# zhouxuguang/GNXRayTracer

Hardware: AMD Instinct MI355X
Metric: Mrays/sec + wall-clock to 1024spp, dragon Cornell 1920×1080 (higher is better)
Workload: dtype f32; 1 GPU; cfg3: Cornell + synthetic 100000-tri mesh (stand-in for absent dragon.3d), Glass+Metal, PathIntegrator maxDepth 8 rr 1 spatial, Halton(1024), 1920x1080; passes_in_flight=4, sub_passes=56, spp_rendered=1024, gather=n/a, world_size=1, backend=none, devices_visible=1

## Files before the change

### gnxraytracer_amd/__init__.py

```python
import collections
import ctypes as C
import os

import numpy as np

from . import _abi
from ._abi import (Camera, Hit, Light, LiSample, Material, Medium, Ray, RenderParams, SceneDesc, Stats, Texture)
from ._tensors import (ANY_GPU, SOME, _addr, _arrays_on_device, _edit_stream, _expect, _got, _host_or_device, _image, _image_size, _is_tensor, _is_torch, _only_kw,
                       _out_tensor, _outputs, _ptr, _refuse, _same_count, _stream_handle, _stream_pair)

_HERE = os.path.dirname(os.path.abspath(__file__))
LIB_PATH = os.environ.get("GNXR_LIB", os.path.join(_HERE, "libgnxr.so"))


class GnxrError(RuntimeError):
    pass


_lib = None
_device = 0


def lib():
    global _lib
# ... 212 lines not shown
        return _check(lib().gnxr_builder_add_sphere(self._h, c, float(radius), int(material), int(medium_inside), int(medium_outside)))

    def set_camera(self, eye=(0, 0, 5), look=(0, 0, 0), up=(0, 1, 0), fov=90.0, lens_radius=0.0, focal_distance=3.0, orthographic=False):
        cam = Camera(_f3(eye), _f3(look), _f3(up), fov, lens_radius, focal_distance, int(bool(orthographic)))
        _check(lib().gnxr_builder_set_camera(self._h, C.byref(cam)))

    def set_bvh_split_method(self, method):
        _check(lib().gnxr_builder_set_bvh_split_method(self._h, {"sah": 0, "hlbvh": 1, "middle": 2, "equal_counts": 3}[method]))

    def set_camera_medium(self, medium):
        _check(lib().gnxr_builder_set_camera_medium(self._h, int(medium)))

    def desc(self):
        d = SceneDesc()
        _check(lib().gnxr_builder_desc(self._h, C.byref(d)))
        return d


def camera(eye=(0, 0, 5), look=(0, 0, 0), up=(0, 1, 0), fov=90.0, lens_radius=0.0, focal_distance=3.0, orthographic=False):
    return Camera(_f3(eye), _f3(look), _f3(up), fov, lens_radius, focal_distance, int(bool(orthographic)))


def _material_albedo(m):
    rgb = (C.c_float * 3)()
    _check(lib().gnxr_material_albedo(C.byref(m), rgb))
    return np.array(rgb[:], dtype=np.float32)


def material_albedo(**material_fields):
    return _material_albedo(material(**material_fields))


def material(**material_fields):
    m = Material()
    for k, v in material_fields.items():
        if isinstance(v, (tuple, list, np.ndarray)):
            setattr(m, k, (C.c_float * len(v))(*[float(x) for x in v]))
        else:
            setattr(m, k, v)
    return m


def write_synthetic_3d(path, target_triangles=100000, seed=1):
    _check(lib().gnxr_write_synthetic_3d(os.fsencode(path), int(target_triangles), int(seed)))


class Scene:

    def __init__(self, builder_or_desc):
        self._h = C.c_void_p()
        self._keep = builder_or_desc
        d = builder_or_desc.desc() if isinstance(builder_or_desc, SceneBuilder) else builder_or_desc
        self.n_triangles = int(d.n_triangles)
        self.n_vertices = int(d.n_vertices)
        self.n_lights = int(d.n_lights)
        self.device = _device
        self.camera = Camera()
        C.memmove(C.byref(self.camera), C.byref(d.camera), C.sizeof(Camera))
        self._env_light = None
        for i in range(int(d.n_lights)):
            if d.lights[i].type == _abi.LIGHT_INFINITE:
                self._env_light = Light()
                C.memmove(C.byref(self._env_light), C.byref(d.lights[i]), C.sizeof(Light))
                break
        self._textures = []
        for i in range(int(d.n_textures)):
            t = Texture()
            C.memmove(C.byref(t), C.byref(d.textures[i]), C.sizeof(Texture))
            t.texel_offset = 0
            self._textures.append(t)
        _check(lib().gnxr_scene_create(C.byref(d), C.byref(self._h)))

    def close(self):
        if getattr(self, "_h", None) and _lib is not None:
            _lib.gnxr_scene_destroy(self._h)
            self._h = None

    __del__ = close

    def info(self):
        n, dmax, nv = C.c_int32(), C.c_int32(), C.c_int32()
        _check(lib().gnxr_scene_info(self._h, C.byref(n), C.byref(dmax), C.byref(nv)))
        return {"bvh_nodes": n.value, "bvh_max_depth": dmax.value, "light_voxels": nv.value}

    def nee_apply_counts(self):
        t, w = C.c_uint64(), C.c_uint64()
        _check(lib().gnxr_scene_nee_apply_counts(self._h, C.byref(t), C.byref(w)))
        return int(t.value), int(w.value)

    def update_vertices(self, xyz, first_vertex=0, stream=None, move_lights=False):
        ptr, xyz, _ = _host_or_device("update_vertices", xyz, np.float32, [(None, 3)], "(n, 3)", self.device)
        stream = _stream_handle("update_vertices", _edit_stream(stream, xyz))
        if move_lights:
            _check(lib().gnxr_scene_update_vertices_ex(self._h, int(first_vertex), int(xyz.shape[0]), _addr(ptr), _abi.UPDATE_MOVE_LIGHTS, _addr(stream)))
        else:
            _check(lib().gnxr_scene_update_vertices(self._h, int(first_vertex), int(xyz.shape[0]), _addr(ptr), _addr(stream)))

    def update_lights(self, lights, first_light=0):
        lights = list(lights)
        for l in lights:
            if not isinstance(l, Light):
                raise ValueError(f"update_lights: lights must be gnxr Light records, got {type(l).__name__}")
        arr = (Light * max(len(lights), 1))(*lights)
        _check(lib().gnxr_scene_update_lights(self._h, int(first_light), len(lights), arr))

    def set_lights(self, lights, stream=None):
        lights = list(lights)
        for l in lights:
            if not isinstance(l, Light):
                raise ValueError(f"set_lights: lights must be gnxr Light records, got {type(l).__name__}")
        handle = _stream_handle("set_lights", stream)
        arr = (Light * max(len(lights), 1))()
        for k, l in enumerate(lights):
            C.memmove(C.byref(arr[k]), C.byref(l), C.sizeof(Light))
        _check(lib().gnxr_scene_set_lights(self._h, arr if lights else None, len(lights), _addr(handle)))
        self.n_lights = len(lights)
        self._env_light = None
        for l in lights:
            if l.type == _abi.LIGHT_INFINITE:
                self._env_light = Light()
                C.memmove(C.byref(self._env_light), C.byref(l), C.sizeof(Light))
                break

    def light_tables(self):
        out = []
        for which, dtype, cols in ((0, np.uint32, _abi.DLIGHT_BYTES // 4), (1, np.int32, 0)):
            n = C.c_int64(0)
            _check(lib().gnxr_scene_light_tables(self._h, which, None, 0, C.byref(n)))
            a = np.zeros(n.value // 4, dtype)
            if n.value:
                _check(lib().gnxr_scene_light_tables(self._h, which, C.c_void_p(a.ctypes.data), n.value, C.byref(n)))
            out.append(a.reshape(-1, cols) if cols else a)
        return tuple(out)

    def update_materials(self, materials, first_material=0):
        materials = list(materials)
        for m in materials:
            if not isinstance(m, Material):
                raise ValueError(f"update_materials: materials must be gnxr Material records, got {type(m).__name__}")
        arr = (Material * max(len(materials), 1))(*materials)
        _check(lib().gnxr_scene_update_materials(self._h, int(first_material), len(materials), arr))

    def set_triangle_materials(self, ids, first_triangle=0, stream=None):
        ptr, ids, _ = _host_or_device("set_triangle_materials", ids, np.int32, [(None,)], "(n,)", self.device)
        stream = _stream_handle("set_triangle_materials", _edit_stream(stream, ids))
        _check(lib().gnxr_scene_set_triangle_materials(self._h, int(first_triangle), int(ids.shape[0]), _addr(ptr), _addr(stream)))

    def triangle_materials(self):
        mat = np.zeros(self.n_triangles, np.int32); cls = np.zeros(self.n_triangles, np.uint8)
        rc = lib().gnxr_scene_triangle_materials(self._h, mat.ctypes.data_as(C.POINTER(C.c_int32)), cls.ctypes.data_as(C.POINTER(C.c_uint8)), self.n_triangles)
        if rc < 0:
            _check(rc)
        return mat, cls

    def update_attributes(self, uv=None, normals=None, tangents=None, first_triangle=0, stream=None):
        name = "update_attributes"
        given = [(what, x, cols) for what, x, cols in (("uv", uv, 6), ("normals", normals, 9), ("tangents", tangents, 9)) if x is not None]
        if not given:
            raise ValueError(f"{name}: none of uv, normals, tangents given")
        on_device = _arrays_on_device(name, given[0][0], given[0][1])
        handle = _stream_handle(name, _edit_stream(stream, given[0][1]))
        ptrs, keep, n = {}, [], None
        for what, x, cols in given:
            ptrs[what], x, _ = _host_or_device(f"{name}: {what}", x, np.float32, [(None, cols)], f"(n, {cols})", self.device, on_device)
            keep.append(x)
            if n is not None and x.shape[0] != n:
# ... 621 lines not shown
NearLists = collections.namedtuple("NearLists", "count records prim dist2 p b1 b2 feature")
NearLists.__doc__ = """Scene.within's and Scene.nearest's result: `count`, int32 (n,) -- within: all triangles inside the radius, never clamped;
nearest: the slots filled --, `records`, the (n, K, 8) float32 gnxr_closest_point records -- per query the first min(count, K) near
triangles in ascending (dist2, prim), then empty slots (prim -1, dist2 +inf, the rest 0) --, and views of it: `prim` (n, K) (int32:
authoring-order triangle), `dist2` (n, K), `p` (n, K, 3), `b1`, `b2` (n, K) and `feature` (n, K) (int32, as in ClosestPoints)."""

SphereCasts = collections.namedtuple("SphereCasts", "records prim t p b1 b2 feature")
SphereCasts.__doc__ = """Scene.sphere_cast's result: `records`, the (n, 8) float32 gnxr_closest_point records with t in the dist2 slot, and views of
it -- `prim` (int32: the authoring-order triangle the ball touches first, -1 without a hit), `t` (the time of impact in units of the
direction, +inf without a hit), `p` (n, 3), `b1`, `b2` and `feature` (int32, as in ClosestPoints): the contact point on that triangle."""

ALL_HITS_MAX = 32
NEAR_MAX = 32
CONTAINS_DIRECTION = (0.8017837, 0.5345225, 0.26726124)


def rays_tensor(o, d, tmax=float("inf")):
    import torch
    o = torch.as_tensor(o, dtype=torch.float32).reshape(-1, 3)
    d = torch.as_tensor(d, dtype=torch.float32, device=o.device).reshape(-1, 3)
    r = torch.zeros((o.shape[0], 8), dtype=torch.float32, device=o.device)
    r[:, 0:3] = o
    r[:, 3] = torch.as_tensor(tmax, dtype=torch.float32, device=o.device)
    r[:, 4:7] = d
    return r


def _view_args(name, cameras, media, width, height):
    if cameras is not None:
        cameras = list(cameras)
        for c in cameras:
            if not isinstance(c, Camera):
                raise ValueError(f"{name}: cameras must be gnxr Camera records (camera(...)), got {type(c).__name__}")
        if media is not None:
            media = [int(m) for m in media]
            if len(media) != len(cameras):
                raise ValueError(f"{name}: {len(media)} media for {len(cameras)} cameras")
    return (cameras, media) + _image_size(name, width, height)


def li_samples(px, py, s, medium=-1):
    import torch
    args = {"px": px, "py": py, "s": s, "medium": medium}
    device = next((a.device for a in args.values() if isinstance(a, torch.Tensor)), torch.device("cpu"))
    cols = []
    for name, a in args.items():
        if isinstance(a, torch.Tensor):
            if a.dtype.is_floating_point or a.dtype.is_complex or a.dtype == torch.bool or a.dim() > 1:
                raise ValueError(f"li_samples: {name} must be an integer tensor of shape (n,) or (), got {a.dtype} {tuple(a.shape)}")
            a = a.to(device=device, dtype=torch.int32)
        elif isinstance(a, (int, np.integer)) and not isinstance(a, bool):
            a = torch.tensor(int(a), dtype=torch.int32, device=device)
        else:
            raise ValueError(f"li_samples: {name} must be an integer or an integer tensor, got {type(a).__name__}")
        cols.append(a.reshape(-1))
    try:
        cols = torch.broadcast_tensors(*cols)
    except RuntimeError as e:
        raise ValueError(f"li_samples: the arguments do not broadcast: {e}") from None
    return torch.stack(cols, dim=1).contiguous()


HIT_DTYPE = np.dtype([("prim", np.int32), ("t", np.float32), ("b0", np.float32), ("b1", np.float32), ("b2", np.float32),
                      ("n", np.float32, 3)])


CLOSEST_DTYPE = np.dtype([("prim", np.int32), ("dist2", np.float32), ("p", np.float32, 3), ("b1", np.float32), ("b2", np.float32),
                          ("feature", np.int32)])


RAY_HIT_DTYPE = np.dtype([("t", np.float32), ("prim", np.int32), ("b1", np.float32), ("b2", np.float32)])


def make_rays(o, d, tmax=np.inf):
    o = np.asarray(o, dtype=np.float32).reshape(-1, 3)
    d = np.asarray(d, dtype=np.float32).reshape(-1, 3)
    r = np.zeros((len(o), 8), dtype=np.float32)
    r[:, 0:3] = o
    r[:, 3] = tmax
    r[:, 4:7] = d
    return r


def stats_dict(s):
    return {k: getattr(s, k) for k, _ in Stats._fields_}


class PathIntegrator:
    integrator = _abi.INTEGRATOR_PATH

    def __init__(self, maxDepth=5, rrThreshold=1.0, lightSampleStrategy="spatial"):
        self.maxDepth = int(maxDepth)
        self.rrThreshold = float(rrThreshold)
        self.strategy = LIGHT_STRATEGIES.get(lightSampleStrategy, _abi.LIGHTS_SPATIAL)

    def params(self, width, height, spp, spp_begin=0, spp_end=0, shard_index=0, shard_count=1, shard_rows=1,
               samples_per_pass=0, passes_in_flight=0):
        return RenderParams(width, height, spp, spp_begin, spp_end, self.maxDepth, self.rrThreshold, self.integrator,
                            self.strategy, shard_index, shard_count, shard_rows, samples_per_pass, getattr(self, "directStrategy", 0),
                            passes_in_flight)

    def Li(self, scene, rays, samples, width, height, spp, out=None, stream=None, **kw):
        import torch
        _expect("Li: rays", rays, torch.float32, (8,))
        _expect("Li: samples", samples, torch.int32, (4,))
        n = rays.shape[0]
        _same_count("Li", None, samples.shape[0], n, "rays", "sample records")
        out = _out_tensor("Li: out", out, (n, 4), torch.float32, rays.device)
        _expect("Li: rays", rays, torch.float32, (8,), scene.device)
        _expect("Li: samples", samples, torch.int32, (4,), scene.device)
        stream, _ = _stream_pair(stream, rays.device)
        p = self.params(width, height, spp, **kw)
        st = Stats()
        _check(lib().gnxr_li_device(scene._h, C.byref(p), _ptr(rays), _ptr(samples), n, _ptr(out), _addr(stream), C.byref(st)))
        return out, stats_dict(st)

    def RenderViews(self, scene, cameras, width, height, spp, media=None, out=None, stream=None, **kw):
        import torch
        cameras, media, width, height = _view_args("RenderViews", list(cameras), media, width, height)
        V = len(cameras)
        out = _out_tensor("RenderViews: out", out, (V, height, width, 4), torch.float32, torch.device("cuda", scene.device))
        stream, _ = _stream_pair(stream, out.device)
        p = self.params(width, height, spp, **kw)
        cams = (Camera * max(V, 1))(*cameras)
        med = (C.c_int32 * max(V, 1))(*media) if media is not None else None
        st = Stats()
        _check(lib().gnxr_render_views_device(scene._h, C.byref(p), cams, med, V, _ptr(out), _addr(stream), C.byref(st)))
        return out, stats_dict(st)

    def RenderAdaptive(self, scene, width, height, spp, threshold, min_spp=16, step_spp=16, floor=0.01, guard=1, out=None, count_out=None, stream=None, **kw):
        import math
        import torch
        width, height, spp, min_spp, step_spp, guard = int(width), int(height), int(spp), int(min_spp), int(step_spp), int(guard)
        threshold, floor = float(threshold), float(floor)
        _image_size("RenderAdaptive", width, height)
        if spp < 1 or not 1 <= min_spp <= spp:
            raise ValueError(f"RenderAdaptive: spp >= 1 and min_spp in [1, spp] are required, got spp = {spp}, min_spp = {min_spp}")
        if step_spp < 1:
            raise ValueError(f"RenderAdaptive: step_spp must be at least 1, got {step_spp}")
        if not 0 <= guard <= 8:
            raise ValueError(f"RenderAdaptive: guard must lie in [0, 8], got {guard}")
        if math.isnan(threshold) or threshold < 0 or math.isnan(floor) or floor < 0:
            raise ValueError(f"RenderAdaptive: threshold and floor must be numbers >= 0, got {threshold} and {floor}")
        _only_kw("RenderAdaptive", kw, ("samples_per_pass", "passes_in_flight"))
        hstream, _, out, count_out = _outputs(stream, torch.device("cuda", scene.device), ("RenderAdaptive: out", out, (height, width, 4), torch.float32),
                                              ("RenderAdaptive: count_out", count_out, (height, width), torch.int32))
        p = self.params(width, height, spp, **kw)
        ap = _abi.AdaptiveParams(C.sizeof(_abi.AdaptiveParams), min_spp, step_spp, guard, threshold, floor)
        info = _abi.AdaptiveInfo(C.sizeof(_abi.AdaptiveInfo), 0, 0, 0)
        st = Stats()
        _check(lib().gnxr_render_adaptive_device(scene._h, C.byref(p), C.byref(ap), _ptr(out), _ptr(count_out), _addr(hstream), C.byref(st), C.byref(info)))
        stats = stats_dict(st)
        stats.update(rounds=info.rounds, samples=info.samples, pixels_at_budget=info.pixels_at_budget)
        return out, count_out, stats

    AOV_CHANNELS = ("albedo", "normal", "shading_normal", "depth", "ids")

    def RenderAOV(self, scene, width, height, spp, cameras=None, media=None, channels=AOV_CHANNELS, out=None, stream=None, **kw):
        import torch
        channels = tuple(channels)
        bad = [c for c in channels if c not in self.AOV_CHANNELS]
        if bad or not channels or len(set(channels)) != len(channels):
            raise ValueError(f"RenderAOV: channels must be a non-empty selection of {self.AOV_CHANNELS}, got {channels}")
        if cameras is None and media is not None:
            raise ValueError("RenderAOV: media goes with cameras; the scene's own camera sits in the scene's camera medium")
        cameras, media, width, height = _view_args("RenderAOV", cameras, media, width, height)
        V = len(cameras) if cameras is not None else 1
        _only_kw("RenderAOV", kw, ("spp_begin", "spp_end", "samples_per_pass"))
        device = torch.device("cuda", scene.device)
        lead = (V,) if cameras is not None else ()
        shapes = {"albedo": (4,), "normal": (4,), "shading_normal": (4,), "depth": (), "ids": (2,)}
        out = dict(out) if out is not None else {}
        extra = [c for c in out if c not in channels]
        if extra:
            raise ValueError(f"RenderAOV: out holds {extra}, which channels does not name")
        hstream, _, *tensors = _outputs(stream, device, *((f"RenderAOV: out[{c!r}]", out.get(c), lead + (height, width) + shapes[c], torch.int32 if c == "ids" else torch.float32)
                                                           for c in channels))
        res = dict(zip(channels, tensors))
        bufs = _abi.AovBuffers(*(_ptr(res.get(c)) for c in self.AOV_CHANNELS))
        p = self.params(width, height, spp, **kw)
        cams = (Camera * V)(*cameras) if cameras else None
        med = (C.c_int32 * V)(*media) if media else None
        st = Stats()
        _check(lib().gnxr_render_aov_device(scene._h, C.byref(p), cams, med, V if cameras is not None else 1, C.byref(bufs), _addr(hstream), C.byref(st)))
        return res, stats_dict(st)

    def RenderDenoised(self, scene, width, height, spp, cameras=None, media=None, normal="shading_normal", stream=None, **denoise_kw):
        import torch
        spp = int(spp)
        if spp < 2 or spp % 2:
            raise ValueError(f"RenderDenoised: spp must be even and at least 2 (the two halves are the variance estimate), got {spp}")
        if normal not in ("shading_normal", "normal"):
            raise ValueError(f"RenderDenoised: normal must be 'shading_normal' or 'normal', got {normal!r}")
        if cameras is None and media is not None:
            raise ValueError("RenderDenoised: media goes with cameras; the scene's own camera sits in the scene's camera medium")
        _only_kw("RenderDenoised", denoise_kw, ("iterations", "sigma_color", "sigma_normal", "sigma_depth", "out"))
        cameras, media, width, height = _view_args("RenderDenoised", cameras, media, width, height)
        device = torch.device("cuda", scene.device)
        hstream, tstream = _stream_pair(stream, device)
        halves, stats = [], []
        for lo, hi in ((0, spp // 2), (spp // 2, spp)):
            if cameras is not None:
                img, st = self.RenderViews(scene, cameras, width, height, spp, media=media, stream=tstream, spp_begin=lo, spp_end=hi)
            else:
                with torch.cuda.stream(tstream):
                    img = torch.zeros((height, width, 4), dtype=torch.float32, device=device)
                st = self.RenderDevice(scene, img.data_ptr(), width, height, spp, stream=hstream, spp_begin=lo, spp_end=hi)
            halves.append(img)
            stats.append(st)
        aov, aov_stats = self.RenderAOV(scene, width, height, spp, cameras=cameras, media=media, channels=("albedo", normal, "depth"), stream=tstream)
        image = denoise(halves[0], halves[1], albedo=aov["albedo"], normal=aov[normal], depth=aov["depth"], stream=tstream, **denoise_kw)
        total = {k: stats[0][k] + stats[1][k] for k in stats[0]}
        total["aov"] = aov_stats
        return image, total

    def RenderFiltered(self, scene, width, height, spp, filter, cameras=None, media=None, accum=None, resume=False, out=None, stream=None, **kw):
        import torch
        _film_record("RenderFiltered", filter, "filter must be")
        if cameras is None and media is not None:
            raise ValueError("RenderFiltered: media goes with cameras; the scene's own camera sits in the scene's camera medium")
        cameras, media, width, height = _view_args("RenderFiltered", cameras, media, width, height)
        if resume and accum is None:
            raise ValueError("RenderFiltered: resume continues an accumulator: pass the tensor of the earlier call as accum")
        _only_kw("RenderFiltered", kw, ("spp_begin", "spp_end", "samples_per_pass", "passes_in_flight"))
        V = len(cameras) if cameras is not None else 1
        shape = ((V,) if cameras is not None else ()) + (height, width, 4)
        given = [("RenderFiltered: accum", accum, shape, torch.float32)] if accum is not None else []
        hstream, *_, out = _outputs(stream, torch.device("cuda", scene.device), *given, ("RenderFiltered: out", out, shape, torch.float32))
        p = self.params(width, height, spp, **kw)
        cams = (Camera * V)(*cameras) if cameras else None
        med = (C.c_int32 * V)(*media) if media else None
        st = Stats()
        _check(lib().gnxr_render_filtered_device(scene._h, C.byref(p), C.byref(filter), cams, med, V, _ptr(out), _ptr(accum), _abi.FILM_CONTINUE if resume else 0,
                                                 _addr(hstream), C.byref(st)))
        return out, stats_dict(st)

    def BakeLightmap(self, scene, lm_uv, width, height, spp, dilate=2, flip=False, medium=-1, out=None, stream=None, **kw):
        import torch
        width, height = _image_size("BakeLightmap", width, height, "atlas")
        if int(dilate) < 0:
            raise ValueError(f"BakeLightmap: dilate must be >= 0, got {dilate}")
        _only_kw("BakeLightmap", kw, ("samples_per_pass", "passes_in_flight"))
        _bake_uv("BakeLightmap", scene, lm_uv)
        hstream, _, out = _outputs(stream, lm_uv.device, ("BakeLightmap: out", out, (height, width, 4), torch.float32))
        p = self.params(width, height, spp, **kw)
        bp = _abi.BakeParams(C.sizeof(_abi.BakeParams), _abi.BAKE_FLIP_NORMALS if flip else 0, int(dilate), int(medium))
        st = Stats()
        _check(lib().gnxr_bake_lightmap_device(scene._h, C.byref(p), C.byref(bp), _ptr(lm_uv), _ptr(out), _addr(hstream), C.byref(st)))
        return out, stats_dict(st)

    def BakeLightProbes(self, scene, positions, spp, width=None, height=None, medium=-1, out=None, stream=None, **kw):
        import torch
        _expect("BakeLightProbes: positions", positions, torch.float32, (3,), scene.device)
        n = positions.shape[0]
        if width is None:
            width = max(1, min(n, 1024))
        width = int(width)
        if height is None:
            height = max(1, -(-n // width)) if width > 0 else 0
        height = int(height)
        if width <= 0 or height <= 0 or width * height < n:
            raise ValueError(f"BakeLightProbes: the {width} x {height} grid of pixels does not hold {n} probes")
        _only_kw("BakeLightProbes", kw, ("samples_per_pass", "passes_in_flight"))
        hstream, _, out = _outputs(stream, positions.device, ("BakeLightProbes: out", out, (n, 9, 4), torch.float32))
        p = self.params(width, height, spp, **kw)
        pp = _abi.LightprobeParams(C.sizeof(_abi.LightprobeParams), 0, int(medium))
        st = Stats()
        _check(lib().gnxr_bake_lightprobes_device(scene._h, C.byref(p), C.byref(pp), _ptr(positions), n, _ptr(out), _addr(hstream), C.byref(st)))
        return out, stats_dict(st)

    def Render(self, scene, width, height, spp, **kw):
        p = self.params(width, height, spp, **kw)
        img = np.zeros((height, width, 4), dtype=np.float32)
        st = Stats()
        _check(lib().gnxr_render(scene._h, C.byref(p), img.ctypes.data_as(C.POINTER(C.c_float)), C.byref(st)))
        return img, stats_dict(st)

    def Reserve(self, scene, width, height, spp, **kw):
        p = self.params(width, height, spp, **kw)
        _check(lib().gnxr_render_reserve(scene._h, C.byref(p)))

    def RenderDevice(self, scene, d_ptr, width, height, spp, stream=None, **kw):
        p = self.params(width, height, spp, **kw)
        st = Stats()
        _check(lib().gnxr_render_device(scene._h, C.byref(p), C.c_void_p(int(d_ptr)),
                                        C.c_void_p(int(stream) if stream else None), C.byref(st)))
        return stats_dict(st)


class VolPathIntegrator(PathIntegrator):
    integrator = _abi.INTEGRATOR_VOLPATH


class WhittedIntegrator(PathIntegrator):
    integrator = _abi.INTEGRATOR_WHITTED

    def __init__(self, maxDepth=5):
        super().__init__(maxDepth, 1.0, "uniform")


class DirectLightingIntegrator(PathIntegrator):
    integrator = _abi.INTEGRATOR_DIRECT

    def __init__(self, strategy="all", maxDepth=5):
        super().__init__(maxDepth, 1.0, "uniform")
        self.directStrategy = {"all": _abi.DIRECT_SAMPLE_ALL, "one": _abi.DIRECT_SAMPLE_ONE}[strategy]


def sample_halton(width, height, px, py, s, dim):
    px = np.ascontiguousarray(px, dtype=np.int32)
    py = np.ascontiguousarray(py, dtype=np.int32)
    s = np.ascontiguousarray(s, dtype=np.int64)
    dim = np.ascontiguousarray(dim, dtype=np.int32)
    out = np.zeros(len(px), dtype=np.float32)
    _check(lib().gnxr_sample_halton(width, height, px.ctypes.data_as(C.POINTER(C.c_int32)),
                                    py.ctypes.data_as(C.POINTER(C.c_int32)), s.ctypes.data_as(C.POINTER(C.c_int64)),
                                    dim.ctypes.data_as(C.POINTER(C.c_int32)), len(px),
                                    out.ctypes.data_as(C.POINTER(C.c_float))))
    return out


def camera_rays(camera, width, height, px, py, s):
    px = np.ascontiguousarray(px, dtype=np.int32)
    py = np.ascontiguousarray(py, dtype=np.int32)
    s = np.ascontiguousarray(s, dtype=np.int64)
    o = np.zeros((len(px), 3), dtype=np.float32)
    d = np.zeros((len(px), 3), dtype=np.float32)
    _check(lib().gnxr_camera_rays(C.byref(camera), width, height, px.ctypes.data_as(C.POINTER(C.c_int32)),
                                  py.ctypes.data_as(C.POINTER(C.c_int32)), s.ctypes.data_as(C.POINTER(C.c_int64)),
                                  len(px), o.ctypes.data_as(C.POINTER(C.c_float)),
                                  d.ctypes.data_as(C.POINTER(C.c_float))))
    return o, d


def camera_rays_device(camera, width, height, px, py, s, medium=-1, stream=None):
    import torch
    for what, x in (("px", px), ("py", py), ("s", s)):
        if not _is_tensor(x, torch.int32, (None,), ANY_GPU if x is px else px.device):
            _refuse(x, f"camera_rays_device: {what} must be a contiguous int32 (n,) tensor on one GPU")
        _same_count("camera_rays_device", what, x.shape[0], px.shape[0], "px", "entries")
    n = px.shape[0]
    if not isinstance(camera, Camera):
        raise ValueError(f"camera_rays_device: camera must be a gnxr Camera record (camera(...)), got {type(camera).__name__}")
    st, _, rays, samples = _outputs(stream, px.device, ("camera_rays_device: rays", None, (n, 8), torch.float32), ("camera_rays_device: samples", None, (n, 4), torch.int32))
    _check(lib().gnxr_camera_rays_device(C.byref(camera), int(medium), int(width), int(height), _ptr(px), _ptr(py), _ptr(s), n, _ptr(rays), _ptr(samples), _addr(st)))
    return rays, samples


def denoise(color, color_b=None, albedo=None, normal=None, depth=None, iterations=5, sigma_color=4.0, sigma_normal=0.25, sigma_depth=0.01, out=None, stream=None):
    import math
    import torch
    shape, V, H, W = _image("denoise", "color", color, size=False)
    for what, x, want in (("color_b", color_b, shape), ("albedo", albedo, shape), ("normal", normal, shape), ("depth", depth, shape[:-1])):
        if x is not None and not _is_tensor(x, torch.float32, want, color.device):
            _refuse(x, f"denoise: {what} must be a contiguous float32 tensor of shape {want} on {color.device}")
    _image_size("denoise", W, H)
    iterations = int(iterations)
    if not 1 <= iterations <= 8:
        raise ValueError(f"denoise: iterations must lie in [1, 8], got {iterations}")
    sigmas = [float(sigma_color), float(sigma_normal), float(sigma_depth)]
    if any(math.isnan(s) or s < 0 for s in sigmas):
        raise ValueError(f"denoise: the sigmas must be numbers >= 0, got {sigmas}")
    hstream, _, out = _outputs(stream, color.device, ("denoise: out", out, shape, torch.float32))
    if V == 0:
        return out
    p = _abi.DenoiseParams(C.sizeof(_abi.DenoiseParams), W, H, V, iterations, *sigmas)
    bufs = _abi.DenoiseBuffers(C.sizeof(_abi.DenoiseBuffers), 0, _ptr(color), _ptr(color_b), _ptr(albedo), _ptr(normal), _ptr(depth))
    _check(lib().gnxr_denoise_device(C.byref(p), C.byref(bufs), _ptr(out), _addr(hstream)))
    return out

# ... 482 lines not shown
```

### gnxraytracer_amd/_abi.py

```python
import ctypes as C

GNXR_ABI_VERSION = 5

OK, ERR_INVALID, ERR_NO_DEVICE, ERR_OOM, ERR_UNSUPPORTED, ERR_IO, ERR_RUNTIME = 0, -1, -2, -3, -4, -5, -6
MAT_NONE, MAT_MATTE, MAT_MIRROR, MAT_GLASS, MAT_METAL, MAT_PLASTIC, MAT_DISNEY = range(7)
LIGHT_AREA_TRI, LIGHT_INFINITE, LIGHT_SKYBOX, LIGHT_POINT, LIGHT_SPOT, LIGHT_DISTANT = 1, 2, 3, 4, 5, 6
INTEGRATOR_PATH, INTEGRATOR_VOLPATH, INTEGRATOR_WHITTED, INTEGRATOR_DIRECT = 0, 1, 2, 3
DIRECT_SAMPLE_ALL, DIRECT_SAMPLE_ONE = 0, 1
LIGHTS_SPATIAL, LIGHTS_UNIFORM, LIGHTS_POWER = 0, 1, 2
MEDIUM_HOMOGENEOUS, MEDIUM_GRID = 1, 2
NEAR_ALL, NEAR_NEAREST = 0, 1
DMEDIUM_BYTES = 128
DLIGHT_BYTES = 112
DTEXTURE_BYTES = 112
UPDATE_MOVE_LIGHTS = 1

f32, i32, u8, i64, u32, u64 = C.c_float, C.c_int32, C.c_uint8, C.c_int64, C.c_uint32, C.c_uint64


class Material(C.Structure):
    _fields_ = [
        ("type", i32), ("has_bump", i32), ("remap_roughness", i32), ("disney_thin", i32),
        ("kd", f32 * 3), ("ks", f32 * 3), ("kr", f32 * 3), ("kt", f32 * 3), ("eta", f32 * 3), ("k", f32 * 3),
        ("sigma", f32), ("urough", f32), ("vrough", f32),
# ... 153 lines not shown


class MotionParams(C.Structure):
    _fields_ = [("struct_size", i32), ("width", i32), ("height", i32), ("n_views", i32)]


class MotionBuffers(C.Structure):
    _fields_ = [("struct_size", i32), ("_pad", i32), ("d_motion", C.c_void_p), ("d_guide", C.c_void_p), ("d_prim", C.c_void_p)]


class TemporalParams(C.Structure):
    _fields_ = [("struct_size", i32), ("width", i32), ("height", i32), ("n_views", i32), ("max_history", i32), ("depth_tol", f32), ("normal_cos", f32)]


class TemporalBuffers(C.Structure):
    _fields_ = [("struct_size", i32), ("_pad", i32), ("d_color", C.c_void_p), ("d_motion", C.c_void_p), ("d_guide", C.c_void_p), ("d_prim", C.c_void_p),
                ("d_hist_color", C.c_void_p), ("d_hist_stat", C.c_void_p), ("d_hist_guide", C.c_void_p), ("d_hist_prim", C.c_void_p),
                ("d_out_color", C.c_void_p), ("d_out_stat", C.c_void_p)]


class HistogramParams(C.Structure):
    _fields_ = [("struct_size", i32), ("width", i32), ("height", i32), ("n_views", i32), ("min_log2", i32)]


class ExposureParams(C.Structure):
    _fields_ = [("struct_size", i32), ("n_views", i32), ("min_log2", i32), ("_pad", i32), ("key", f32), ("low", f32), ("high", f32), ("rate", f32),
                ("min_exposure", f32), ("max_exposure", f32)]


class TonemapParams(C.Structure):
    _fields_ = [("struct_size", i32), ("width", i32), ("height", i32), ("n_views", i32), ("curve", i32), ("flags", u32), ("exposure", f32), ("white", f32)]


HISTOGRAM_WORDS = 260
TONEMAP_LINEAR, TONEMAP_REFERENCE, TONEMAP_REINHARD, TONEMAP_ACES = range(4)
TONEMAP_SRGB, TONEMAP_ROUND = 1, 2

class SkinParams(C.Structure):
    _fields_ = [("struct_size", i32), ("n_vertices", i32), ("n_bones", i32), ("n_morphs", i32)]


NORMALS_FLIP = 1

FILTER_BOX, FILTER_TRIANGLE, FILTER_GAUSSIAN, FILTER_MITCHELL, FILTER_TABLE = range(5)
FILM_CONTINUE = 1

P = C.POINTER
VP = C.c_void_p

PROTOTYPES = {
    "gnxr_abi_version": (C.c_int, []),
    "gnxr_abi_sizeof": (C.c_int, [C.c_int]),
    "gnxr_init": (C.c_int, [C.c_int]),
    "gnxr_shutdown": (None, []),
    "gnxr_last_error": (C.c_char_p, []),
    "gnxr_init_devices": (C.c_int, [i32, P(i32)]),
    "gnxr_set_profiling": (C.c_int, [C.c_int]),
    "gnxr_probe_valu_peak": (C.c_int, [P(C.c_double)]),
    "gnxr_probe_gather_peak": (C.c_int, [P(C.c_double)]),
    "gnxr_scene_create": (C.c_int, [P(SceneDesc), P(VP)]),
    "gnxr_scene_destroy": (None, [VP]),
    "gnxr_scene_info": (C.c_int, [VP, P(i32), P(i32), P(i32)]),
    "gnxr_scene_update_vertices": (C.c_int, [VP, i32, i32, VP, VP]),
    "gnxr_scene_update_vertices_ex": (C.c_int, [VP, i32, i32, VP, u32, VP]),
    "gnxr_scene_update_lights": (C.c_int, [VP, i32, i32, P(Light)]),
    "gnxr_scene_set_lights": (C.c_int, [VP, P(Light), i32, VP]),
    "gnxr_scene_light_tables": (C.c_int, [VP, i32, VP, i64, P(i64)]),
    "gnxr_scene_rebuild_bvh": (C.c_int, [VP, VP]),
    "gnxr_scene_set_geometry": (C.c_int, [VP, P(Geometry), VP]),
    "gnxr_scene_update_environment": (C.c_int, [VP, P(Light), VP, i32, i32, VP]),
    "gnxr_scene_env_tables": (C.c_int, [VP, i32, VP, i64, P(i64)]),
    "gnxr_scene_update_media": (C.c_int, [VP, i32, i32, P(Medium), VP, VP]),
    "gnxr_scene_media_tables": (C.c_int, [VP, i32, i32, VP, i64, P(i64)]),
    "gnxr_scene_update_textures": (C.c_int, [VP, i32, i32, P(Texture), VP, VP]),
    "gnxr_scene_texture_tables": (C.c_int, [VP, i32, i32, VP, i64, P(i64)]),
    "gnxr_scene_update_materials": (C.c_int, [VP, i32, i32, P(Material)]),
    "gnxr_scene_set_triangle_materials": (C.c_int, [VP, i32, i32, VP, VP]),
    "gnxr_scene_triangle_materials": (C.c_int, [VP, P(i32), P(C.c_uint8), C.c_int64]),
    "gnxr_scene_set_camera": (C.c_int, [VP, P(Camera), i32]),
    "gnxr_render": (C.c_int, [VP, P(RenderParams), P(f32), P(Stats)]),
    "gnxr_render_device": (C.c_int, [VP, P(RenderParams), VP, VP, P(Stats)]),
    "gnxr_render_reserve": (C.c_int, [VP, P(RenderParams)]),
    "gnxr_scene_nee_apply_counts": (C.c_int, [VP, P(u64), P(u64)]),
    "gnxr_trace_closest": (C.c_int, [VP, P(Ray), i64, P(Hit)]),
    "gnxr_trace_any": (C.c_int, [VP, P(Ray), i64, P(u8)]),
    "gnxr_trace_closest_device": (C.c_int, [VP, VP, i64, VP, VP]),
    "gnxr_trace_any_device": (C.c_int, [VP, VP, i64, VP, VP]),
    "gnxr_closest_point_device": (C.c_int, [VP, VP, i64, VP, VP]),
    "gnxr_closest_point_counted_device": (C.c_int, [VP, VP, i64, VP, VP, VP]),
    "gnxr_closest_point": (C.c_int, [VP, P(PointQuery), i64, P(ClosestPoint)]),
    "gnxr_trace_all_device": (C.c_int, [VP, VP, i64, i32, VP, VP, VP]),
    "gnxr_trace_all_counted_device": (C.c_int, [VP, VP, i64, i32, VP, VP, VP, VP]),
    "gnxr_trace_all": (C.c_int, [VP, P(Ray), i64, i32, P(RayHit), P(i32)]),
    "gnxr_near_device": (C.c_int, [VP, VP, i64, i32, u32, VP, VP, VP]),
    "gnxr_near_counted_device": (C.c_int, [VP, VP, i64, i32, u32, VP, VP, VP, VP]),
    "gnxr_near": (C.c_int, [VP, P(PointQuery), i64, i32, u32, P(ClosestPoint), P(i32)]),
    "gnxr_sphere_cast_device": (C.c_int, [VP, VP, i64, VP, VP]),
    "gnxr_sphere_cast_counted_device": (C.c_int, [VP, VP, i64, VP, VP, VP]),
    "gnxr_sphere_cast": (C.c_int, [VP, P(SphereCast), i64, P(ClosestPoint)]),
    "gnxr_li_device": (C.c_int, [VP, P(RenderParams), VP, VP, i64, VP, VP, P(Stats)]),
    "gnxr_render_views_device": (C.c_int, [VP, P(RenderParams), P(Camera), P(i32), i32, VP, VP, P(Stats)]),
    "gnxr_render_aov_device": (C.c_int, [VP, P(RenderParams), P(Camera), P(i32), i32, P(AovBuffers), VP, P(Stats)]),
    "gnxr_render_adaptive_device": (C.c_int, [VP, P(RenderParams), P(AdaptiveParams), VP, VP, VP, P(Stats), P(AdaptiveInfo)]),
    "gnxr_denoise_device": (C.c_int, [P(DenoiseParams), P(DenoiseBuffers), VP, VP]),
    "gnxr_film_filter_table": (C.c_int, [P(FilmFilter), P(f32)]),
    "gnxr_film_add_device": (C.c_int, [P(FilmFilter), i32, i32, i32, i32, VP, VP, VP, VP]),
    "gnxr_film_resolve_device": (C.c_int, [i32, i32, i32, VP, VP, VP]),
    "gnxr_render_filtered_device": (C.c_int, [VP, P(RenderParams), P(FilmFilter), P(Camera), P(i32), i32, VP, VP, u32, VP, P(Stats)]),
    "gnxr_bake_texels_device": (C.c_int, [VP, VP, i32, i32, VP, VP, VP]),
    "gnxr_surface_rays_device": (C.c_int, [VP, i32, i32, VP, VP, VP, VP, VP, i64, u32, i32, VP, VP, VP, VP]),
    "gnxr_bake_dilate_device": (C.c_int, [i32, i32, i32, VP, VP]),
    "gnxr_bake_lightmap_device": (C.c_int, [VP, P(RenderParams), P(BakeParams), VP, VP, VP, P(Stats)]),
    "gnxr_lightprobe_rays_device": (C.c_int, [VP, i32, i32, VP, VP, VP, VP, i64, i32, VP, VP, VP]),
    "gnxr_sh_project_device": (C.c_int, [VP, VP, i32, i64, VP, u32, VP]),
    "gnxr_bake_lightprobes_device": (C.c_int, [VP, P(RenderParams), P(LightprobeParams), VP, i32, VP, VP, P(Stats)]),
    "gnxr_sh_irradiance_device": (C.c_int, [VP, i32, VP, VP, i64, VP, VP]),
    "gnxr_camera_matrices": (C.c_int, [P(Camera), i32, i32, P(f32), P(f32), P(f32)]),
    "gnxr_motion_device": (C.c_int, [VP, P(MotionParams), P(Camera), P(Camera), VP, P(MotionBuffers), VP]),
    "gnxr_temporal_accumulate_device": (C.c_int, [P(TemporalParams), P(TemporalBuffers), VP]),
    "gnxr_luminance_histogram_device": (C.c_int, [P(HistogramParams), VP, VP, VP]),
    "gnxr_exposure_device": (C.c_int, [P(ExposureParams), VP, VP, VP, VP]),
    "gnxr_tonemap_device": (C.c_int, [P(TonemapParams), VP, VP, VP, VP]),
    "gnxr_scene_update_attributes": (C.c_int, [VP, i32, i32, VP, VP, VP, VP]),
    "gnxr_scene_triangle_attributes": (C.c_int, [VP, i32, P(f32), i64, P(i64)]),
    "gnxr_scene_recompute_normals": (C.c_int, [VP, u32, VP]),
    "gnxr_skin_vertices_device": (C.c_int, [P(SkinParams), VP, VP, VP, VP, VP, VP, VP, VP]),
    "gnxr_material_albedo": (C.c_int, [P(Material), P(f32)]),
    "gnxr_camera_rays_device": (C.c_int, [P(Camera), i32, i32, i32, VP, VP, VP, i64, VP, VP, VP]),
    "gnxr_bsdf_device": (C.c_int, [VP, VP, VP, VP, VP, i64, i32, VP, VP]),
    "gnxr_light_sample_device": (C.c_int, [VP, VP, i64, i32, VP, VP]),
    "gnxr_light_le_device": (C.c_int, [VP, i32, VP, i64, VP, VP]),
    "gnxr_sample_halton": (C.c_int, [i32, i32, P(i32), P(i32), P(i64), P(i32), i64, P(f32)]),
    "gnxr_camera_rays": (C.c_int, [P(Camera), i32, i32, P(i32), P(i32), P(i64), i64, P(f32), P(f32)]),
    "gnxr_framebuffer_update": (C.c_int, [P(f32), P(f32), i32, i32, i32, P(u8)]),
    "gnxr_framebuffer_save_png": (C.c_int, [C.c_char_p, P(u8), i32, i32]),
    "gnxr_light_grid_table": (C.c_int, [VP, i32, i32, P(f32), i64, P(i64)]),
    "gnxr_eval_libm": (C.c_int, [i32, P(f32), P(f32), i64, P(f32)]),
    "gnxr_eval_libm_f64": (C.c_int, [i32, P(f32), i64, P(C.c_double)]),
    "gnxr_builder_create": (C.c_int, [P(VP)]),
    "gnxr_builder_set_camera_medium": (C.c_int, [VP, i32]),
    "gnxr_builder_add_sphere": (C.c_int, [VP, P(f32), f32, i32, i32, i32]),
    "gnxr_builder_destroy": (None, [VP]),
    "gnxr_builder_add_material": (C.c_int, [VP, P(Material)]),
    "gnxr_builder_matte": (C.c_int, [VP, P(f32), f32]),
    "gnxr_builder_mirror": (C.c_int, [VP, P(f32)]),
    "gnxr_builder_purple_plastic": (C.c_int, [VP]),
    "gnxr_builder_yellow_metal": (C.c_int, [VP]),
    "gnxr_builder_white_glass": (C.c_int, [VP]),
    "gnxr_builder_add_mesh": (C.c_int, [VP, P(f32), i32, P(i32), i32, P(f32), i32, i32, i32]),
    "gnxr_builder_add_model_3d": (C.c_int, [VP, C.c_char_p, i32]),
    "gnxr_builder_add_cornell": (C.c_int, [VP, i32, i32, i32]),
    "gnxr_builder_add_floor": (C.c_int, [VP, i32]),
    "gnxr_builder_add_area_light": (C.c_int, [VP, i32]),
    "gnxr_builder_add_sky_light": (C.c_int, [VP]),
    "gnxr_builder_add_inf_light": (C.c_int, [VP, C.c_char_p]),
    "gnxr_builder_add_inf_light_data": (C.c_int, [VP, P(f32), i32, i32, P(f32), P(f32)]),
    "gnxr_builder_add_medium": (C.c_int, [VP, P(Medium), P(f32)]),
    "gnxr_builder_add_volume_file": (C.c_int, [VP, C.c_char_p, f32, f32, P(f32)]),
    "gnxr_builder_add_emissive_mesh": (C.c_int, [VP, P(f32), i32, P(i32), i32, P(f32), i32, P(f32), i32]),
    "gnxr_builder_add_spot_light": (C.c_int, [VP]),
    "gnxr_builder_add_dist_light": (C.c_int, [VP]),
    "gnxr_builder_add_light": (C.c_int, [VP, P(Light)]),
    "gnxr_builder_add_texture_data": (C.c_int, [VP, P(Texture), P(f32), i32, i32]),
    "gnxr_builder_add_texture_file": (C.c_int, [VP, P(Texture), C.c_char_p]),
    "gnxr_builder_set_material_texture": (C.c_int, [VP, i32, i32, i32]),
    "gnxr_builder_set_triangle_uv": (C.c_int, [VP, i32, i32, P(f32)]),
# ... 22 lines not shown
```

### gnxraytracer_amd/csrc/api.hip

```cpp
#include <hip/hip_runtime.h>

#include <chrono>
#include <cstdio>
#include <cstdlib>
#include <memory>
#include <mutex>
#include <string>
#include <thread>
#include <vector>

#include "host_scene.h"
#include "kernels.hip.h"
#include "trace4_kernel.hip.h"
#include "hlbvh_build.hip.h"
#include "refit_kernel.hip.h"
#include "material_kernel.hip.h"
#include "rebuild_kernel.hip.h"
#include "geometry_kernel.hip.h"
#include "lights_kernel.hip.h"
#include "env_build_kernel.hip.h"
#include "media_kernel.hip.h"
#include "texture_build_kernel.hip.h"
#include "li_kernel.hip.h"
#include "views_kernel.hip.h"
// ... 101 lines not shown
    return GNXR_OK;
}
#endif
#ifdef GX_TAIL_STAMP
int gnxr_debug_tail_stamp(unsigned long long *out12, int reset) {
    if (hipMemcpyFromSymbol(out12, HIP_SYMBOL(g_tail), 12 * sizeof(unsigned long long)) != hipSuccess) return GNXR_ERR_INVALID;
    if (reset) { unsigned long long z[12] = {~0ull, 0ull, ~0ull, 0ull}; (void)hipMemcpyToSymbol(HIP_SYMBOL(g_tail), z, sizeof(z)); }
    return GNXR_OK;
}
#endif

static int upload_scene(gnxr_scene *s, const SceneUploadTables &up) {
    const SceneFacts &cs = s->cs;
    int rc;
    if (cs.bvh_max_depth + 1 > 64) { set_error("BVH depth %d exceeds the 64-entry traversal stack (BVHAccel.cpp:661)", cs.bvh_max_depth); return GNXR_ERR_UNSUPPORTED; }
    s->set_traversal(std::any_of(up.nodes.begin(), up.nodes.end(), [](const DNode &n) { return (n.meta & 0xffffu) > 127; }));
#define UP(from, field) if ((rc = s->field.upload(from.field)) != GNXR_OK) return rc;
    UP(up, nodes) UP(up, nodes4) UP(up, tris) UP(up, leaf_boxes) UP(up, tri_class) UP(cs, lights) UP(cs, perms) UP(cs, primes) UP(cs, prime_sums) UP(cs, prime_magic)
    UP(cs, dmedia) UP(up, grid_density) UP(up, tri_media) UP(cs, spheres) UP(cs, textures) UP(up, tex_texels) UP(up, ewa_lut) UP(up, tri_uv) UP(up, tri_n) UP(up, tri_s)
    UP(cs, aov_albedo)
    UP(cs, env_texels4) UP(cs, env_cond_func) UP(cs, env_cond_cdf) UP(cs, env_cond_int) UP(cs, env_marg_func) UP(cs, env_marg_cdf) UP(cs, env_marg_guide) UP(cs, env_cond_guide)
#undef UP
    {
        const size_t worst = 2 * cs.desc_materials.size();
        if ((rc = s->material_authored.alloc(worst)) || (rc = s->materials.alloc(1 + worst)) || (rc = s->materials_single.alloc(1 + worst))) return rc;
        if ((rc = s->material_authored.upload(cs.material_authored)) != GNXR_OK) return rc;
        const DTexTables at = s->tex_tables(s->tri_uv.p, s->tri_n.p, s->tri_s.p);
        if ((rc = s->write_material_tables(cs.materials, cs.materials_single, at.tri_uv, at.tri_n, at.tri_s)) != GNXR_OK) return rc;
    }
    if ((rc = s->infinite.upload(cs.infinite_lights)) != GNXR_OK) return rc;
    if ((rc = s->counters.alloc(1)) != GNXR_OK) return rc;
    if (hipHostMalloc((void **)&s->h_counters, sizeof(Counters)) != hipSuccess) { set_error("hipHostMalloc failed"); return GNXR_ERR_OOM; }
    if (hipHostMalloc((void **)&s->h_ring, sizeof(Counters) * gnxr_scene::kRing) != hipSuccess) { set_error("hipHostMalloc failed"); return GNXR_ERR_OOM; }
    for (hipEvent_t &e : s->ring_ev) HIP_TRY(hipEventCreateWithFlags(&e, hipEventDisableTiming));
    for (hipStream_t &a : s->aux_stream) HIP_TRY(hipStreamCreateWithFlags(&a, hipStreamNonBlocking));
    HIP_TRY(hipEventCreateWithFlags(&s->ev_fork, hipEventDisableTiming));
    for (hipEvent_t &e : s->ev_join) HIP_TRY(hipEventCreateWithFlags(&e, hipEventDisableTiming));
    return GNXR_OK;
}

int gnxr_scene_create(const gnxr_scene_desc *desc, gnxr_scene **out) {
    if (!desc || !out) { set_error("null argument"); return GNXR_ERR_INVALID; }
    int rc = ensure_device();
    if (rc) return rc;
    gnxr_scene *s = new (std::nothrow) gnxr_scene(g_device);
    if (!s) return GNXR_ERR_OOM;
    CompiledScene compiled;
    if (!compile_scene(desc, &compiled, device_hlbvh_build)) { delete s; return GNXR_ERR_INVALID; }
    s->cs = std::move(static_cast<SceneFacts &>(compiled));
    s->cs.refit_seeds = std::move(static_cast<RefitSeeds &>(compiled));
    for (size_t i = 1; i < g_devices.size(); ++i) s->replicas.push_back(std::make_unique<gnxr_scene>(g_devices[i], s->host));
    s->host->copies_awaiting_seeds = s->n_copies();
    if ((rc = s->each_copy([&](gnxr_scene *c, size_t) { return upload_scene(c, compiled); })) != GNXR_OK) { delete s; return rc; }
    const SceneFacts &cs = s->cs;
    if (getenv("GNXR_VERBOSE"))
        fprintf(stderr, "[gnxr] scene: %zu tris, %zu nodes (depth %d), %zu 4-wide nodes (stack %d), wide=%d, %zu device(s)\n", cs.n_triangles, cs.n_nodes, cs.bvh_max_depth,
                cs.n_nodes4, cs.stack4_need, (int)s->wide_ok, s->n_copies());
    *out = s;
    return GNXR_OK;
}
void gnxr_scene_destroy(gnxr_scene *s) { delete s; }

int gnxr_scene_info(const gnxr_scene *s, int32_t *n_nodes, int32_t *max_depth, int32_t *n_vox) {
    if (!s) return GNXR_ERR_INVALID;
    if (n_nodes) *n_nodes = (int32_t)s->cs.n_nodes;
    if (max_depth) *max_depth = s->cs.bvh_max_depth;
    if (n_vox) *n_vox = s->grid_strategy >= 0 ? s->grid.nvox[0] * s->grid.nvox[1] * s->grid.nvox[2] : 0;
    return GNXR_OK;
}

int gnxr_scene_nee_apply_counts(gnxr_scene *s, uint64_t *in_trace, uint64_t *by_sweep) {
    if (!s) { set_error("null argument"); return GNXR_ERR_INVALID; }
    std::lock_guard<std::recursive_mutex> lock(s->render_mutex);
    uint64_t t = 0, w = 0;
    for (size_t i = 0; i <= s->replicas.size(); ++i) {
        const Counters *c = s->copy(i)->h_counters;
        if (c) { t += c->nee_applied_trace; w += c->nee_applied_sweep; }
    }
    if (in_trace) *in_trace = t;
    if (by_sweep) *by_sweep = w;
    return GNXR_OK;
}

int gnxr_render_device(gnxr_scene *s, const gnxr_render_params *pin, void *d_rgba_out, void *hip_stream, gnxr_stats *stats) {
    return render_sharded(s, pin, d_rgba_out, hip_stream, stats);
}

int gnxr_render_reserve(gnxr_scene *s, const gnxr_render_params *pin) {
    if (!s || !pin) { set_error("null argument"); return GNXR_ERR_INVALID; }
    int dummy = 0;
    return render_sharded(s, pin, &dummy, nullptr, nullptr, true);
}

int gnxr_render(gnxr_scene *s, const gnxr_render_params *p, float *rgba_out, gnxr_stats *stats) {
    if (!s || !p || !rgba_out) { set_error("null argument"); return GNXR_ERR_INVALID; }
    if (p->width <= 0 || p->height <= 0) { set_error("invalid image size"); return GNXR_ERR_INVALID; }
    size_t npx = (size_t)p->width * p->height;
    std::lock_guard<std::recursive_mutex> lock(s->render_mutex);
    if (int brc = s->bind()) return brc;
    const bool grew = !(s->out.p && npx <= s->out.n);
    int rc = s->out.alloc(npx);
    if (rc) return rc;
    HIP_TRY(hipMemset(s->out.p, 0, npx * sizeof(float4)));
    rc = render_sharded(s, p, s->out.p, nullptr, stats);
    if (rc) { if (grew) s->out.release(); return rc; }
    int sc = p->shard_count > 0 ? p->shard_count : 1, sr = p->shard_rows > 0 ? p->shard_rows : 1;
    if (sc == 1) {
        HIP_TRY(hipMemcpy(rgba_out, s->out.p, npx * sizeof(float4), hipMemcpyDeviceToHost));
    } else {
        for (int y = 0; y < p->height; ++y)
            if ((y / sr) % sc == p->shard_index)
                HIP_TRY(hipMemcpy(rgba_out + (size_t)y * p->width * 4, s->out.p + (size_t)y * p->width, (size_t)p->width * sizeof(float4), hipMemcpyDeviceToHost));
    }
    return GNXR_OK;
}

int gnxr_scene_bvh(const gnxr_scene *sc, float *bounds6, int32_t *meta3, int32_t *ordered, int64_t node_capacity, int64_t *n_nodes) {
    if (!sc || !n_nodes) { set_error("bad argument"); return GNXR_ERR_INVALID; }
    gnxr_scene *s = const_cast<gnxr_scene *>(sc);
    std::lock_guard<std::recursive_mutex> lock(s->render_mutex);
    *n_nodes = (int64_t)s->cs.n_nodes;
    if (!bounds6 || !meta3 || !ordered || node_capacity < *n_nodes) return GNXR_OK;
    if (int rc = s->bind()) return rc;
    std::vector<DNode> nodes(s->cs.n_nodes);
    std::vector<DTri> tris(s->cs.n_triangles);
    HIP_TRY(hipMemcpy(nodes.data(), s->nodes.p, nodes.size() * sizeof(DNode), hipMemcpyDeviceToHost));
    HIP_TRY(hipMemcpy(tris.data(), s->tris.p, tris.size() * sizeof(DTri), hipMemcpyDeviceToHost));
    for (size_t i = 0; i < nodes.size(); ++i) {
        const DNode &n = nodes[i];
        bounds6[6 * i + 0] = n.lo[0]; bounds6[6 * i + 1] = n.lo[1]; bounds6[6 * i + 2] = n.lo[2];
        bounds6[6 * i + 3] = n.hi0; bounds6[6 * i + 4] = n.hi1; bounds6[6 * i + 5] = n.hi2;
        const int nPrims = (int)(n.meta & 0xffffu);
        meta3[3 * i + 0] = n.offset; meta3[3 * i + 1] = nPrims; meta3[3 * i + 2] = nPrims ? 0 : (int)(n.meta >> 16);
    }
    for (size_t i = 0; i < tris.size(); ++i) ordered[i] = tris[i].prim;
    return GNXR_OK;
}

int gnxr_trace_closest(gnxr_scene *s, const gnxr_ray *rays, int64_t n, gnxr_hit *hits) {
    if (!s || !rays || !hits || n < 0) { set_error("bad argument"); return GNXR_ERR_INVALID; }
    if (n == 0) return GNXR_OK;
    if (int brc = s->bind()) return brc;
    DevBuf<gnxr_ray> dr;
    DevBuf<gnxr_hit> dh;
    int rc;
    if ((rc = dr.upload(rays, (size_t)n)) || (rc = dh.alloc((size_t)n))) return rc;
    DScene sc = s->device_scene(1, 1);
    if ((rc = binary_trace_api(s, sc, dr.p, n, dh.p, false, nullptr)) != GNXR_OK) return rc;
    HIP_TRY(hipMemcpy(hits, dh.p, (size_t)n * sizeof(gnxr_hit), hipMemcpyDeviceToHost));
    return GNXR_OK;
}
int gnxr_trace_any(gnxr_scene *s, const gnxr_ray *rays, int64_t n, uint8_t *occluded) {
    if (!s || !rays || !occluded || n < 0) { set_error("bad argument"); return GNXR_ERR_INVALID; }
    if (n == 0) return GNXR_OK;
    if (int brc = s->bind()) return brc;
    DevBuf<gnxr_ray> dr;
    DevBuf<unsigned char> dob;
    int rc;
    if ((rc = dr.upload(rays, (size_t)n)) || (rc = dob.alloc((size_t)n))) return rc;
    DScene sc = s->device_scene(1, 1);
    if ((rc = binary_trace_api(s, sc, dr.p, n, dob.p, true, nullptr)) != GNXR_OK) return rc;
    HIP_TRY(hipMemcpy(occluded, dob.p, (size_t)n, hipMemcpyDeviceToHost));
    return GNXR_OK;
}

}
// ... 186 lines not shown
```

### gnxraytracer_amd/csrc/api_common.hip.h

```cpp
#pragma once

namespace { int hip_status(hipError_t e); }
#define HIP_TRY(expr)                                                                                   \
    do {                                                                                                \
        hipError_t e_ = (expr);                                                                         \
        if (e_ != hipSuccess) {                                                                         \
            set_error("%s failed: %s (%s:%d)", #expr, hipGetErrorString(e_), __FILE__, __LINE__);       \
            return hip_status(e_);                                                                      \
        }                                                                                               \
    } while (0)

namespace {

int hip_status(hipError_t e) {
    if (e == hipErrorOutOfMemory) return GNXR_ERR_OOM;
    if (e == hipErrorNoDevice || e == hipErrorInvalidDevice || e == hipErrorInsufficientDriver || e == hipErrorNotInitialized) return GNXR_ERR_NO_DEVICE;
    return GNXR_ERR_RUNTIME;
}

int g_device = -1;
std::vector<int> g_devices;
std::vector<char> g_peer_ok;
int g_num_cus = 256;
int g_profiling = 0;
int g_grid_bpc = 8;
int g_trace_blocks_per_cu = 5;

struct KernelTimer {
    std::vector<hipEvent_t> pool;
    struct Span { int kind; hipEvent_t a, b; };
    std::vector<Span> open;
    size_t used = 0;
    double seconds[3] = {0, 0, 0};
    unsigned launches[3] = {0, 0, 0};
    hipEvent_t get() {
        if (used == pool.size()) { hipEvent_t e; if (hipEventCreate(&e) != hipSuccess) return nullptr; pool.push_back(e); }
        return pool[used++];
    }
    void begin(int kind, hipStream_t st) { Span s{kind, get(), get()}; if (s.a && s.b) { (void)hipEventRecord(s.a, st); open.push_back(s); } }
    void end(hipStream_t st) { if (!open.empty()) (void)hipEventRecord(open.back().b, st); }
    void collect() {
        for (auto &s : open) { float ms = 0; if (hipEventElapsedTime(&ms, s.a, s.b) == hipSuccess) { seconds[s.kind] += ms * 1e-3; launches[s.kind]++; } }
        open.clear();
        used = 0;
    }
    ~KernelTimer() { for (auto e : pool) (void)hipEventDestroy(e); }
};

struct Knobs {
    static int env_int(const char *name, int unset) { const char *e = getenv(name); return e ? atoi(e) : unset; }
    static bool env_set(const char *name) { return getenv(name) != nullptr; }
#define GX_ONCE(type, expr) do { static const type v = (expr); return v; } while (0)
    static int trace_blocks_per_cu() { const int v = env_int("GNXR_TRACE_BLOCKS_PER_CU", 0); return v >= 1 && v <= 8 ? v : 0; }
    static int grid_blocks_per_cu() { const int v = env_int("GNXR_GRID_BLOCKS_PER_CU", 0); return v >= 1 && v <= 4096 ? v : 0; }
    static int trace_lds_levels() { GX_ONCE(int, env_set("GNXR_TRACE_LDS_LEVELS") ? std::max(2, env_int("GNXR_TRACE_LDS_LEVELS", 0)) : 64); }
    static int trace_chunk() { GX_ONCE(int, env_set("GNXR_TRACE_CHUNK") ? std::max(64, env_int("GNXR_TRACE_CHUNK", 0) / 64 * 64) : kTraceChunk); }
    static bool leaf_box_table() { GX_ONCE(bool, env_set("GNXR_LEAF_BOX_TABLE")); }
    static int regions() { GX_ONCE(int, env_int("GNXR_REGIONS", 0)); }
    static bool pipeline() { GX_ONCE(bool, env_int("GNXR_PIPELINE", 1) != 0); }
    static int pipe_cut() { GX_ONCE(int, env_int("GNXR_PIPE_CUT", -1)); }
    static int loop_lag() { GX_ONCE(int, env_int("GNXR_LOOP_LAG", -1)); }
    static int shade_blocks_per_cu() { GX_ONCE(int, env_set("GNXR_SHADE_BLOCKS_PER_CU") ? std::max(1, env_int("GNXR_SHADE_BLOCKS_PER_CU", 0)) : 32); }
    static int shade_lds_dims() { GX_ONCE(int, env_set("GNXR_SHADE_LDS_DIMS") ? std::max(0, std::min(128, env_int("GNXR_SHADE_LDS_DIMS", 0))) : 64); }
    static bool shade_lds_tables() { GX_ONCE(bool, env_int("GNXR_SHADE_LDS_TABLES", 1) != 0); }
    static int shade_streams() { GX_ONCE(int, env_int("GNXR_SHADE_STREAMS", -1)); }
    static bool vol_pack() { GX_ONCE(bool, env_int("GNXR_VOL_PACK", 1) != 0); }
#undef GX_ONCE
    static int volmedia_step_cap() { return env_set("GNXR_VOLMEDIA_STEP_CAP") ? std::max(0, env_int("GNXR_VOLMEDIA_STEP_CAP", 0)) : 64; }
    static bool no_escape_queue() { return env_set("GNXR_NO_ESCAPE_QUEUE"); }
    static bool no_material_queues() { return env_set("GNXR_NO_MATERIAL_QUEUES"); }
    static bool no_narrow_shade() { return env_set("GNXR_NO_NARROW_SHADE"); }
    static bool no_mis_defer() { return env_set("GNXR_NO_MIS_DEFER"); }
    static int mis_defer_step() { const int v = env_int("GNXR_MIS_DEFER_STEP", 2); return v == 1 ? 1 : 2; }
    static int mis_defer_drain_at() { return std::max(1, std::min(64, env_int("GNXR_MIS_DEFER_DRAIN_AT", 64))); }
    static bool no_trace_nee_apply() { return env_set("GNXR_NO_TRACE_NEE_APPLY"); }
    static bool host_light_grid() { return env_set("GNXR_HOST_LIGHT_GRID"); }
    static bool binary_bvh() { return env_set("GNXR_BINARY_BVH"); }
    static long long closest_bin_min() { const char *e = getenv("GNXR_CLOSEST_BIN_MIN"); return e ? std::max(1ll, atoll(e)) : 65536ll; }
    static int closest_lds_levels() { return std::max(1, std::min(24, env_int("GNXR_CLOSEST_LDS_LEVELS", 16))); }
    static int allhits_lds_levels() { return std::max(1, std::min(32, env_int("GNXR_ALLHITS_LDS_LEVELS", 16))); }
    static int near_lds_levels() { return std::max(1, std::min(24, env_int("GNXR_NEAR_LDS_LEVELS", 16))); }
    static int spherecast_lds_levels() { return std::max(1, std::min(24, env_int("GNXR_SPHERECAST_LDS_LEVELS", 16))); }
};

int ensure_device() {
    if (g_device >= 0) { HIP_TRY(hipSetDevice(g_device)); return GNXR_OK; }
    int n = 0;
    hipError_t e = hipGetDeviceCount(&n);
    if (e != hipSuccess || n <= 0) {
        set_error("no HIP device available (%s); libgnxr has no CPU fallback", e != hipSuccess ? hipGetErrorString(e) : "0 devices");
        return GNXR_ERR_NO_DEVICE;
    }
    int dev = 0;
    HIP_TRY(hipGetDevice(&dev));
    hipDeviceProp_t prop;
    HIP_TRY(hipGetDeviceProperties(&prop, dev));
    g_num_cus = prop.multiProcessorCount > 0 ? prop.multiProcessorCount : 256;
    g_device = dev;
    if (const int v = Knobs::trace_blocks_per_cu()) g_trace_blocks_per_cu = v;
    if (const int v = Knobs::grid_blocks_per_cu()) g_grid_bpc = v;
    return GNXR_OK;
}

template <typename T>
struct DevBuf {
    T *p = nullptr;
    size_t n = 0;
    ~DevBuf() { release(); }
    void release() { if (p) { (void)hipFree(p); p = nullptr; n = 0; } }
    int alloc(size_t count) {
        if (count <= n && p) return GNXR_OK;
        release();
        if (count == 0) count = 1;
        HIP_TRY(hipMalloc((void **)&p, count * sizeof(T)));
        n = count;
        return GNXR_OK;
    }
    int upload(const T *src, size_t count) {
        int rc = alloc(count);
        if (rc) return rc;
        if (count) HIP_TRY(hipMemcpy(p, src, count * sizeof(T), hipMemcpyHostToDevice));
        return GNXR_OK;
    }
    template <typename V> int upload(const V &v) { return upload(v.data(), v.size()); }
};

int grid_for(long long n, int blocks_per_cu = 0) {
    if (blocks_per_cu <= 0) blocks_per_cu = g_grid_bpc;
    long long need = (n + kBlock - 1) / kBlock;
    long long cap = (long long)g_num_cus * blocks_per_cu;
    return (int)std::max<long long>(1, std::min(need, cap));
}

}
```

### gnxraytracer_amd/csrc/api_render.hip.h

```cpp
#pragma once

struct TraceLaunch {
    int entries;
    int lds_entries;
    bool spill_needed;
    size_t lds;
    int n_top;
    int blocks;
};
static TraceLaunch trace_launch(const gnxr_scene *s, bool wide, bool spheres, long long total) {
    TraceLaunch t;
    t.entries = wide ? s->cs.stack4_need + 1 : s->cs.bvh_max_depth + 2;
    const int per_cu = g_trace_blocks_per_cu;
    const size_t fixed_b = wide ? (size_t)(kRayRecDwords + (spheres ? 1 : 0)) * kRqStride * sizeof(int) + (size_t)kTopCache * 128 + kOrderTableBytes : 0;
    t.lds_entries = std::min(std::min(t.entries, Knobs::trace_lds_levels()), std::max(2, (int)(((160 * 1024) / per_cu - 1024 - fixed_b) / (kBlock * sizeof(int)))));
    t.spill_needed = t.entries > t.lds_entries;
    t.lds = (size_t)t.lds_entries * kBlock * sizeof(int) + fixed_b;
    t.n_top = (int)std::min<size_t>(kTopCache, s->cs.root4 >= 0 ? s->cs.n_nodes4 : 0);
    t.blocks = (int)std::min<long long>((long long)g_num_cus * per_cu, (total + kBlock - 1) / kBlock);
    return t;
}

static int count_local_rows(const gnxr_render_params *p) {
    int rows = 0;
// ... 254 lines not shown
    const size_t max_tiles = (std::max(cap, pl.pixel_list ? (size_t)pl.npix : (size_t)0) + kCompactTile - 1) / kCompactTile;
    if (tile_desc.n < kCompactMaxOut * max_tiles || !tile_desc.p) {
        if ((rc = tile_desc.alloc(kCompactMaxOut * max_tiles)) != GNXR_OK) return rc;
        HIP_TRY(hipMemset(tile_desc.p, 0, tile_desc.n * sizeof(unsigned long long)));
        HIP_TRY(hipDeviceSynchronize());
        compact_seq = 0;
    }
    if ((rc = compact_ticket.alloc(2)) != GNXR_OK) return rc;
    if (pl.n_views > 0 && (rc = view_cams.alloc((size_t)pl.n_views)) != GNXR_OK) return rc;
    return GNXR_OK;
}

unsigned long long RenderState::state_bytes(const RenderPlan &pl) {
    const unsigned long long per_slot = (2ull * kRecGroups + 2) * sizeof(float4) + 8ull * sizeof(int) + 2 + sizeof(unsigned int);
    const unsigned long long tiles = ((unsigned long long)pl.cap + kCompactTile - 1) / kCompactTile;
    return (unsigned long long)pl.cap * per_slot + tiles * kCompactMaxOut * sizeof(unsigned long long) +
           (pl.volpath ? (unsigned long long)pl.cap * (6ull * sizeof(float4) + sizeof(int4) + 1) : 0ull);
}

PathArrays RenderState::path_arrays() {
    PathArrays pa;
    float4 *rec_primary[kRecGroups];
    record_ptrs(rec, rec_primary);
    pa.bind_records(rec_primary);
    pa.mis_Y = mis_Y.p;
    pa.L = L.p; pa.hit = hit.p; pa.pflags = pflags.p; pa.pclass = pclass.p; pa.nee_vis = nee_vis.p;
    return pa;
}
VolArrays RenderState::vol_arrays() {
    VolArrays va;
    float4 *rec_primary[kRecGroups];
    record_ptrs(rec, rec_primary);
    va.bind_records(rec_primary);
    va.mis_Y = mis_Y.p;
    va.vs = vol_vs.p; va.n1 = vol_n1.p; va.f = vol_f.p;
    va.Li = vol_Li.p; va.Tr = vol_Tr.p; va.Ld = vol_Ld.p; va.mres = vol_mres.p; va.state = vol_state.p;
    va.orig = vol_orig.p; va.Lout = vol_Lout.p;
    return va;
}
WhittedArrays RenderState::whitted_arrays(const RenderPlan &pl, int n_lights) {
    WhittedArrays wa;
    wa.ws = vol_vs.p; wa.fr_o = wh_o.p; wa.fr_d = wh_d.p; wa.fr_L = wh_L.p; wa.fr_w = wh_w.p; wa.fr_pdf = wh_pdf.p;
    wa.fr_rxo = wh_rxo.p; wa.fr_rxd = wh_rxd.p; wa.fr_ryo = wh_ryo.p; wa.fr_ryd = wh_ryd.p;
    wa.cap = (int)pl.cap; wa.n_lights = n_lights; wa.n_records = pl.n_records;
    wa.start_dim = pl.wmode == WM_DIRECT_ALL ? 5 + 2 * (pl.p.max_depth * n_lights * 2) : 5;
    return wa;
}
VolPackSet RenderState::pack_set(bool alt) {
    VolPackSet ps;
    if (!alt) {
        float4 *a[kVolPackF4] = {L.p, reinterpret_cast<float4 *>(vol_vs.p), vol_n1.p, vol_f.p, vol_Li.p, vol_Tr.p, vol_Ld.p, mis_Y.p, vol_mres.p};
        for (int i = 0; i < kVolPackF4; ++i) ps.f4[i] = a[i];
        record_ptrs(rec, ps.rec);
        ps.state = vol_state.p; ps.orig = vol_orig.p;
    } else {
        for (int i = 0; i < kVolPackF4; ++i) ps.f4[i] = vol_alt[i].p;
        record_ptrs(vol_alt_rec, ps.rec);
        ps.state = vol_alt_state.p; ps.orig = vol_alt_orig.p;
    }
    return ps;
}

struct RenderRun {
    gnxr_scene *s;
    RenderState &st;
    hipStream_t stream;
    const RenderPlan &pl;
    const RaySource *src;
    const ViewSource *views;
    const PixelListSource *pix;
    const FilmSource *film = nullptr;
    float4 *film_accum = nullptr;
    DScene sc;
    DRender r;
    PathArrays pa;
    VolArrays va;
    WhittedArrays wa;
    DMediaTables mt;
    Counters *dctr;
    KernelTimer timer;
    const bool timing = (g_profiling & 1) != 0, count_wide = (g_profiling & 4) != 0, counting = (g_profiling & 2) != 0 && !count_wide;
    bool spheres;
    const int mis_mode = Knobs::no_mis_defer() ? 0 : Knobs::mis_defer_step(), mis_drain_at = Knobs::mis_defer_drain_at();
    bool list_media = false;
    int n_lights, n_scene_media;
    unsigned long long rays_closest = 0, rays_any = 0, rays_mis = 0, media_segments = 0;
    unsigned long long new_paths = 0;
    unsigned int launches = 0, passes = 0, loop_iterations = 0;

    RenderRun(gnxr_scene *scene, hipStream_t stream_, const RenderPlan &plan, const RaySource *src_, const ViewSource *views_, const PixelListSource *pix_, const DScene &sc_,
              const DRender &r_)
        : s(scene), st(scene->st), stream(stream_), pl(plan), src(src_), views(views_), pix(pix_), sc(sc_), r(r_), pa(st.path_arrays()), va(st.vol_arrays()),
          wa(st.whitted_arrays(plan, (int)scene->cs.desc_lights.size())), mt(scene->media_tables()), dctr(scene->counters.p), spheres(scene->cs.n_spheres > 0),
          n_lights((int)scene->cs.desc_lights.size()), n_scene_media((int)scene->cs.media.size()) {}

    void launch_trace(TraceWork w, int n_sh, int n_mis, bool count_rays = true);
    void compact(int mode, const int *qin, int nin, const unsigned char *keys, int nout, int nscatter, unsigned int *totals, int *o0, int *o1, int *o2, int *o3 = nullptr, int split = 0,
                 const unsigned *n_dev = nullptr, unsigned kind_queue = 0x01010101u);
    int shade_stage(const int *q_in, int n, int *q_out, const unsigned *n_dev);
    void raygen(const PathArrays &at, long long u0, int kk, unsigned char *medium_keys);
    void resolve(const PathArrays &at, long long u0, int kk);
    void bind_set(const VolPackSet &ps);
};

void RenderRun::launch_trace(TraceWork w, int n_sh, int n_mis, bool count_rays) {
    long long total = (long long)w.n_closest + w.n_nee;
    if (total <= 0) return;
    w.order = nullptr;
    (void)hipMemsetAsync(&dctr->cursor, 0, sizeof(unsigned int), stream);
    const bool wide = s->wide_ok && !counting;
    const TraceLaunch tl = trace_launch(s, wide, spheres, total);
    if (timing) timer.begin(0, stream);
    const int chunk = Knobs::trace_chunk();
#define GX_TRACE(C, W, S) hipLaunchKernelGGL((k_trace<C, W, S>), dim3(tl.blocks), dim3(kBlock), tl.lds, stream, sc, pa, w, &dctr->cursor, dctr, tl.lds_entries, st.trace_spill.p, chunk)
#define GX_TRACE4(C, S, P) hipLaunchKernelGGL((k_trace4<C, S, P>), dim3(tl.blocks), dim3(kBlock), tl.lds, stream, sc, pa, w, &dctr->cursor, dctr, tl.lds_entries, st.trace_spill.p, chunk, tl.n_top)
#define GX_TRACE4_CS(C, S) do { if (tl.spill_needed) GX_TRACE4(C, S, true); else GX_TRACE4(C, S, false); } while (0)
    if (wide) {
        if (spheres) { if (count_wide) GX_TRACE4_CS(true, true); else GX_TRACE4_CS(false, true); }
        else { if (count_wide) GX_TRACE4_CS(true, false); else GX_TRACE4_CS(false, false); }
    } else {
        const bool cnt = counting || count_wide;
        if (spheres) { if (cnt) GX_TRACE(true, false, true); else GX_TRACE(false, false, true); }
        else { if (cnt) GX_TRACE(true, false, false); else GX_TRACE(false, false, false); }
    }
#undef GX_TRACE4_CS
#undef GX_TRACE4
#undef GX_TRACE
    if (timing) timer.end(stream);
    if (count_rays) {
        rays_closest += (unsigned long long)w.n_closest + (unsigned long long)n_mis;
        rays_any += (unsigned long long)n_sh;
        rays_mis += (unsigned long long)n_mis;
    }
    ++launches;
}

void RenderRun::compact(int mode, const int *qin, int nin, const unsigned char *keys, int nout, int nscatter, unsigned int *totals, int *o0, int *o1, int *o2, int *o3, int split,
                        const unsigned *n_dev, unsigned kind_queue) {
    const int tiles = (nin + kCompactTile - 1) / kCompactTile;
    const int g = std::max(1, std::min(tiles, g_num_cus * kCompactBlocksPerCu));
    if (st.compact_seq >= (1u << 30) - 1u) {
        (void)hipMemsetAsync(st.tile_desc.p, 0, st.tile_desc.n * sizeof(unsigned long long), stream);
        st.compact_seq = 0;
    }
    const unsigned seq = ++st.compact_seq;
    const CompactScratch cs{st.tile_desc.p, tiles, st.compact_ticket.p + (seq & 1u), st.compact_ticket.p + ((seq + 1u) & 1u), seq};
    const bool hitclass = mode == COMPACT_HITCLASS;
    const int *hit = hitclass ? (const int *)st.hit.p : nullptr;
    const unsigned char *cls = hitclass ? (const unsigned char *)s->tri_class.p : nullptr;
#define GX_COMPACT(M, N, NS) hipLaunchKernelGGL((k_compact<M, N, NS>), dim3(g), dim3(kCompactBlock), 0, stream, qin, nin, keys, cs, totals, o0, o1, o2, o3, hit, cls, kind_queue, split, n_dev, dctr)
    if (mode == COMPACT_FLAGS) {
        if (nout == 5) { if (nscatter == 3) GX_COMPACT(COMPACT_FLAGS, 5, 3); else GX_COMPACT(COMPACT_FLAGS, 5, 2); }
        else { if (nscatter == 3) GX_COMPACT(COMPACT_FLAGS, 4, 3); else GX_COMPACT(COMPACT_FLAGS, 4, 2); }
    } else if (hitclass) { if (nout == 4) GX_COMPACT(COMPACT_HITCLASS, 4, 4); else GX_COMPACT(COMPACT_HITCLASS, 3, 3); }
    else if (nout == 4) GX_COMPACT(COMPACT_CLASS, 4, 4);
    else GX_COMPACT(COMPACT_CLASS, 3, 3);
#undef GX_COMPACT
    launches += 1;
}
static int compact_stalled(const Counters &c) {
    if (!c.compact_stall) return GNXR_OK;
    set_error("queue compaction: a tile waited for its predecessors beyond the poll limit (k_compact); the render was abandoned");
    return GNXR_ERR_RUNTIME;
}

constexpr size_t kShadeLdsBudget = 52 * 1024;

int RenderRun::shade_stage(const int *q_in, int n, int *q_out, const unsigned *n_dev) {
    if (timing) timer.begin(2, stream);
    const int *qk = pl.queue_kernel;
    const int n_classes = qk[3] != SHADE_Q_NONE ? 4 : 3;
    compact(COMPACT_HITCLASS, q_in, n, st.pclass.p, n_classes, n_classes, &dctr->q_class[0], st.queue_c0.p, st.queue_c1.p, st.queue_c2.p, st.queue_c3.p, 0, n_dev, pl.kind_queue);
    int *qc[4] = {st.queue_c0.p, st.queue_c1.p, st.queue_c2.p, st.queue_c3.p};
    dim3 g(grid_for(n, Knobs::shade_blocks_per_cu())), b(kBlock);
    const int sdims = std::min<int>(Knobs::shade_lds_dims(), (int)s->cs.prime_sums.size() - 1);
    const int snperm = sdims > 0 ? s->cs.prime_sums[sdims] : 0;
    const bool shade_lds_tabs = Knobs::shade_lds_tables();
    const int lmats = (shade_lds_tabs && s->cs.materials.size() <= 12) ? (int)s->cs.materials.size() : 0;
    const int llights = (shade_lds_tabs && n_lights > 0 && n_lights <= 16) ? n_lights : 0;
    const size_t slds = (sdims > 0 ? ((((size_t)snperm * 2 + 15) & ~(size_t)15) + (size_t)sdims * 32) : 0) + (size_t)lmats * sizeof(DMaterial) + (size_t)llights * sizeof(DLight);
    const int shade_streams = Knobs::shade_streams();
    int n_class_kernels = 0;
    for (int q = 0; q < 4; ++q) n_class_kernels += qk[q] != SHADE_Q_NONE ? 1 : 0;
    const bool fork = (shade_streams < 0 ? n_class_kernels >= 3 : (shade_streams != 0 && n_class_kernels >= 2)) && s->aux_stream[0] && s->aux_stream[1];
    hipStream_t cst[4] = {stream, stream, stream, stream};
    if (fork) {
        HIP_TRY(hipEventRecord(s->ev_fork, stream));
        HIP_TRY(hipStreamWaitEvent(s->aux_stream[0], s->ev_fork, 0));
        HIP_TRY(hipStreamWaitEvent(s->aux_stream[1], s->ev_fork, 0));
        cst[1] = s->aux_stream[0]; cst[2] = s->aux_stream[1]; cst[3] = s->aux_stream[1];
    }
    const bool area_only = pl.area_only, area_env_only = pl.area_env_only;
#define GX_SHADE_KA(K, C, LDS, LL) hipLaunchKernelGGL(K, g, b, LDS, cst[C], sc, r, pa, (const int *)qc[C], (const unsigned int *)&dctr->q_class[C], sdims, snperm, lmats, LL)
#define GX_SHADE_K(K, C) GX_SHADE_KA(K, C, slds, llights)
#define GX_SHADE(LMV, LTV, C) do { if (spheres) GX_SHADE_K((k_shade<LMV, LTV, true>), C); else GX_SHADE_K((k_shade<LMV, LTV, false>), C); } while (0)
#define GX_SHADE_AREA_S(LMV, SPHV, C) do { \
        if (mis_step == 2) GX_SHADE_KA((k_shade<LMV, LT_AREA | SM_DEFER, SPHV>), C, slds_mis, llights_mis); \
        else if (mis_step == 1) GX_SHADE_K((k_shade<LMV, LT_AREA | SM_DIR_FIRST, SPHV>), C); \
        else GX_SHADE_K((k_shade<LMV, LT_AREA, SPHV>), C); } while (0)
#define GX_SHADE_AREA(LMV, C) do { if (spheres) GX_SHADE_AREA_S(LMV, true, C); else GX_SHADE_AREA_S(LMV, false, C); } while (0)
#define GX_SHADE_TEX(LTV) do { if (spheres) GX_SHADE_K((k_shade<LM_ALL, LTV, true, true>), 3); else GX_SHADE_K((k_shade<LM_ALL, LTV, false, true>), 3); } while (0)
    const int light_set = area_only ? 0 : ((area_env_only && !spheres && !(pl.class_mask & 8)) ? 1 : 2);
    int mis_step = light_set == 0 ? mis_mode : 0;
    const size_t slds_mis = slds + (size_t)(kBlock / 64) * ((size_t)kMisEntryWords * kMisCap + 1) * sizeof(int);
    const int llights_mis = llights | (std::min(mis_drain_at, kMisCap) << 8);
    if (mis_step == 2 && slds_mis > kShadeLdsBudget) mis_step = 1;
#define GX_SHADE_LM(LMV, C) do { \
        if (light_set == 0) GX_SHADE_AREA(LMV, C); \
        else if (light_set == 1) GX_SHADE_K((k_shade<LMV, LT_AREA | LT_ENV, false>), C); \
        else GX_SHADE(LMV, LT_ALL, C); } while (0)
#define GX_SHADE_NARROW(LMV, C) do { \
        if (light_set == 0) GX_SHADE_AREA_S(LMV, false, C); \
        else if (light_set == 1) GX_SHADE_K((k_shade<LMV, LT_AREA | LT_ENV, false>), C); \
        else GX_SHADE_K((k_shade<LMV, LT_ALL, false>), C); } while (0)
    for (int q = 0; q < 4; ++q) {
        switch (qk[q]) {
        case SHADE_Q_DIFFUSE: GX_SHADE_LM(LM_DIFFUSE, q); break;
        case SHADE_Q_GLOSSY: GX_SHADE_LM(LM_GLOSSY, q); break;
        case SHADE_Q_CONDUCTOR: GX_SHADE_NARROW(LM_CONDUCTOR, q); break;
        case SHADE_Q_ROUGH_DIELECTRIC: GX_SHADE_NARROW(LM_ROUGH_DIELECTRIC, q); break;
        case SHADE_Q_ALL: GX_SHADE_LM(LM_ALL, q); break;
        case SHADE_Q_TEX: if (light_set == 0) GX_SHADE_TEX(LT_AREA); else GX_SHADE_TEX(LT_ALL); break;
        case SHADE_Q_ESCAPE:
            if (area_env_only) hipLaunchKernelGGL((k_shade_escape<LT_AREA | LT_ENV>), g, b, 0, cst[q], sc, pa, (const int *)qc[q], (const unsigned int *)&dctr->q_class[q]);
            else hipLaunchKernelGGL((k_shade_escape<LT_ALL>), g, b, 0, cst[q], sc, pa, (const int *)qc[q], (const unsigned int *)&dctr->q_class[q]);
            break;
        default: continue;
        }
        ++launches;
    }
#undef GX_SHADE_NARROW
#undef GX_SHADE_LM
#undef GX_SHADE_TEX
#undef GX_SHADE_AREA
#undef GX_SHADE_AREA_S
#undef GX_SHADE
#undef GX_SHADE_K
#undef GX_SHADE_KA
    if (fork) {
        HIP_TRY(hipEventRecord(s->ev_join[0], s->aux_stream[0]));
        HIP_TRY(hipEventRecord(s->ev_join[1], s->aux_stream[1]));
        HIP_TRY(hipStreamWaitEvent(stream, s->ev_join[0], 0));
        HIP_TRY(hipStreamWaitEvent(stream, s->ev_join[1], 0));
    }
    compact(COMPACT_FLAGS, q_in, n, st.pflags.p, 4, 2, &dctr->q_next, q_out, st.queue_nee.p, nullptr, nullptr, 0, n_dev);
    if (timing) timer.end(stream);
    return GNXR_OK;
}

void RenderRun::raygen(const PathArrays &at, long long u0, int kk, unsigned char *medium_keys) {
    const int n_new = (int)(pl.unit * kk);
    if (pix) hipLaunchKernelGGL(k_raygen_pixels, dim3(grid_for(n_new)), dim3(kBlock), 0, stream, sc, r, at, pix->round, n_new, u0);
    else if (views) hipLaunchKernelGGL(k_raygen_views, dim3(grid_for(n_new)), dim3(kBlock), 0, stream, sc, r, (const DCamera *)st.view_cams.p, at, n_new, (int)u0, medium_keys);
    else if (!src) hipLaunchKernelGGL(k_raygen, dim3(grid_for(n_new)), dim3(kBlock), 0, stream, sc, r, at, n_new, (int)u0);
    else hipLaunchKernelGGL(k_raygen_rays, dim3(grid_for(n_new)), dim3(kBlock), 0, stream, sc, r, at, reinterpret_cast<const float4 *>(src->rays + u0),
                            reinterpret_cast<const int4 *>(src->samples + u0), n_new, n_scene_media, medium_keys, dctr, u0);
}
void RenderRun::resolve(const PathArrays &at, long long u0, int kk) {
    if (pix) hipLaunchKernelGGL(k_adaptive_accum, dim3(grid_for(pix->round.n_active)), dim3(kBlock), 0, stream, (const float4 *)at.L, pix->round, kk, u0, st.accum.p, st.ad_A.p);
    else if (film) {
        const FilmImage im = film_image(r.W, r.H, std::max(1, pl.n_views));
        hipLaunchKernelGGL(k_film_add<true>, dim3(film_grid(im)), dim3(kBlock), 0, stream, im, film->f, film->tab, (const float4 *)at.L, (const float2 *)nullptr, sc.st, (int)u0, kk, film_accum);
    }
    else if (!src) hipLaunchKernelGGL(k_resolve, dim3(grid_for(r.npix)), dim3(kBlock), 0, stream, at, st.accum.p, r.npix, kk);
    else hipLaunchKernelGGL(k_store_li, dim3(grid_for(kk)), dim3(kBlock), 0, stream, (const float4 *)at.L, reinterpret_cast<const int4 *>(src->samples + u0), r,
                            n_scene_media, kk, reinterpret_cast<float4 *>(src->L) + u0);
}
void RenderRun::bind_set(const VolPackSet &ps) {
    pa.bind_records(ps.rec); va.bind_records(ps.rec);
    pa.L = ps.f4[0]; va.vs = reinterpret_cast<int4 *>(ps.f4[1]); va.n1 = ps.f4[2]; va.f = ps.f4[3]; va.Li = ps.f4[4]; va.Tr = ps.f4[5]; va.Ld = ps.f4[6]; pa.mis_Y = va.mis_Y = ps.f4[7]; va.mres = ps.f4[8];
    va.state = ps.state; va.orig = ps.orig;
}

#define GX_CHECK_LAUNCHES(where)                                                                                    \
    do {                                                                                                            \
        const hipError_t le_ = hipGetLastError();                                                                   \
        if (le_ != hipSuccess) { set_error("HIP runtime error in " where ": %s", hipGetErrorString(le_)); return hip_status(le_); } \
    } while (0)

static int run_path_loop(RenderRun &run) {
    gnxr_scene *s = run.s;
    RenderState &st = run.st;
    const RenderPlan &pl = run.pl;
    hipStream_t stream = run.stream;
    Counters *dctr = run.dctr;
    const size_t half = pl.half;
    struct Sub { long long u0; int kk; };
    std::vector<Sub> subs;
    for (long long u0 = pl.unit_begin; u0 < pl.unit_end; u0 += pl.k) subs.push_back(Sub{u0, (int)std::min<long long>(pl.k, pl.unit_end - u0)});
    const int R = pl.in_flight;
    struct Region { int sub = -1, started = -1; long long paths = 0; } reg[kMaxRegions];
    const int lag = std::max(1, std::min(gnxr_scene::kRing - 2, Knobs::loop_lag() >= 0 ? Knobs::loop_lag() : 2));
    const int stagger = Knobs::pipe_cut() >= 0 ? Knobs::pipe_cut() : std::max(1, (pl.p.max_depth + 2 + lag + R - 1) / R);
    int *qbuf[2] = {st.queue_a.p, st.queue_b.p};
    int in_idx = 0;
    const int nee_in_trace = Knobs::no_trace_nee_apply() ? 0 : 1;
    const unsigned *cnt_ptr = &dctr->n_queue;
    size_t next_sub = 0, done_subs = 0;
    int iter = 0, last_start = -(1 << 20), newest_seen = -1;
    int ring_iter[gnxr_scene::kRing];
    for (int &v : ring_iter) v = -1;
    Counters seen;
    memset(&seen, 0, sizeof(seen));
    long long guard = 0;
    while (done_subs < subs.size()) {
        {
            int oldest_needed = iter - 1 - lag;
            for (int j = newest_seen + 1; j <= oldest_needed; ++j) {
                const int slot = j % gnxr_scene::kRing;
                if (j >= 0 && ring_iter[slot] == j) HIP_TRY(hipEventSynchronize(s->ring_ev[slot]));
            }
            for (int j = iter - 1; j > newest_seen; --j) {
                const int slot = ((j % gnxr_scene::kRing) + gnxr_scene::kRing) % gnxr_scene::kRing;
                if (j < 0 || ring_iter[slot] != j) continue;
                const hipError_t q = hipEventQuery(s->ring_ev[slot]);
                if (q == hipSuccess) { seen = s->h_ring[slot]; newest_seen = j; if (int rc = compact_stalled(seen)) return rc; break; }
                if (q != hipErrorNotReady) { set_error("HIP runtime error in the path loop: hipEventQuery: %s", hipGetErrorString(q)); return hip_status(q); }
                (void)hipGetLastError();
            }
        }
        for (bool progress = true; progress;) {
            progress = false;
            for (int rg = 0; rg < R; ++rg) {
                Region &g = reg[rg];
                if (g.sub >= 0 && (run.src || g.sub == (int)done_subs) && newest_seen > g.started && seen.region_alive[rg] == 0) {
                    run.resolve(run.pa.at((size_t)rg * half), subs[g.sub].u0, subs[g.sub].kk);
                    ++run.launches; ++run.passes; ++done_subs;
                    g.sub = -1;
                    progress = true;
                }
            }
        }
        if (done_subs == subs.size()) break;
        bool any_active = false;
        long long n_upper = 0;
        for (int rg = 0; rg < R; ++rg) {
            const Region &g = reg[rg];
            if (g.sub < 0) continue;
            any_active = true;
            n_upper += newest_seen > g.started ? std::min<long long>(g.paths, seen.region_alive[rg]) : g.paths;
        }
        const int out_idx = 1 - in_idx;
        if (any_active) {
            if (int rc = run.shade_stage(qbuf[in_idx], (int)n_upper, qbuf[out_idx], cnt_ptr)) return rc;
            hipLaunchKernelGGL(k_loop_tail, dim3(1), dim3(64), 0, stream, (const int *)qbuf[out_idx], dctr, R, (int)half, (unsigned)iter);
            ++run.launches;
            const int slot = iter % gnxr_scene::kRing;
            HIP_TRY(hipMemcpyAsync(&s->h_ring[slot], dctr, sizeof(Counters), hipMemcpyDeviceToHost, stream));
            HIP_TRY(hipEventRecord(s->ring_ev[slot], stream));
            ring_iter[slot] = iter;
        }
        int trace_idx = out_idx;
        long long n_trace_upper = n_upper;
        int free_rg = -1;
        for (int rg = 0; rg < R && free_rg < 0; ++rg) if (reg[rg].sub < 0) free_rg = rg;
        const bool start = next_sub < subs.size() && free_rg >= 0 && (!any_active || iter - last_start >= stagger);
        if (start) {
            const Sub &nw = subs[next_sub];
            const int n_new = (int)(pl.unit * nw.kk);
            const size_t base = (size_t)free_rg * half;
            run.raygen(run.pa.at(base), nw.u0, nw.kk, nullptr);
            hipLaunchKernelGGL(k_queue_merge, dim3(grid_for(n_upper + n_new)), dim3(kBlock), 0, stream, (const int *)qbuf[out_idx], dctr, any_active ? 0 : 1, free_rg, (int)base, n_new, qbuf[in_idx]);
            run.launches += 2;
            trace_idx = in_idx; n_trace_upper = n_upper + n_new;
            run.new_paths += (unsigned long long)n_new;
            reg[free_rg].sub = (int)next_sub; reg[free_rg].started = iter; reg[free_rg].paths = n_new;
            last_start = iter;
            ++next_sub;
        }
        if (any_active || start) {
            TraceWork tw{qbuf[trace_idx], (int)n_trace_upper, st.queue_nee.p, any_active ? (int)n_upper : 0, nullptr, reinterpret_cast<unsigned char *>(st.nee_vis.p), cnt_ptr,
                         any_active ? (const unsigned *)&dctr->q_nee : nullptr, nee_in_trace};
            run.launch_trace(tw, 0, 0, false);
            if (any_active) {
                if (run.timing) run.timer.begin(1, stream);
                hipLaunchKernelGGL(k_nee_combine, dim3(grid_for(n_upper)), dim3(kBlock), 0, stream, run.pa, (const int *)st.queue_nee.p, (int)n_upper, reinterpret_cast<const unsigned char *>(st.nee_vis.p),
                                   (const unsigned *)&dctr->q_nee, &dctr->nee_applied_sweep);
                if (run.timing) run.timer.end(stream);
                ++run.launches;
            }
            in_idx = trace_idx;
        }
        GX_CHECK_LAUNCHES("the path loop");
        ++iter; ++run.loop_iterations;
        if (++guard > (1ll << 24)) { set_error("path loop did not terminate"); return GNXR_ERR_INVALID; }
    }
    return GNXR_OK;
}

static int run_whitted_pass(RenderRun &run, long long u0, int kk) {
    RenderState &st = run.st;
    const RenderPlan &pl = run.pl;
    hipStream_t stream = run.stream;
    Counters *dctr = run.dctr;
    const DScene &sc = run.sc;
    const DRender &r = run.r;
    const PathArrays &pa = run.pa;
    const WhittedArrays &wa = run.wa;
    const int n_paths = (int)(pl.unit * kk), n_records = pl.n_records;
    const bool textured = pl.textured_scene;
    hipLaunchKernelGGL(k_whitted_init, dim3(grid_for(n_paths)), dim3(kBlock), 0, stream, pa, wa, n_paths);
    ++run.launches;
    if (textured) {
        if (run.views) hipLaunchKernelGGL(k_whitted_init_diff_views, dim3(grid_for(n_paths)), dim3(kBlock), 0, stream, sc, r, (const DCamera *)st.view_cams.p, pa, wa, n_paths);
        else hipLaunchKernelGGL(k_whitted_init_diff, dim3(grid_for(n_paths)), dim3(kBlock), 0, stream, sc, r, pa, wa, n_paths);
        ++run.launches;
    }
    int n = n_paths, n_cl = n_paths, n_shp = 0, guard = 0;
    const int *q_in = nullptr, *q_cl = nullptr;
    int *q_cur = st.queue_a.p, *q_other = st.queue_b.p;
    unsigned long long *d_shadow = &dctr->whitted_shadow;
    while (n > 0) {
        if (n_shp > 0) {
            hipLaunchKernelGGL(k_whitted_expand, dim3(grid_for((long long)n_shp * n_records)), dim3(kBlock), 0, stream, (const int *)st.queue_nee.p, n_shp, n_records, (int)pl.cap, st.wh_rec.p);
            ++run.launches;
        }
        run.launch_trace(TraceWork{q_cl, n_cl, st.wh_rec.p, n_shp * n_records}, 0, 0);
        if (run.timing) run.timer.begin(2, stream);
#define GX_WH2(MODEV, LTV, SPHV)                                                                                                                     \
    do {                                                                                                                                             \
        if (textured) hipLaunchKernelGGL((k_whitted_step<MODEV, LTV, SPHV, true>), dim3(grid_for(n)), dim3(kBlock), 0, stream, sc, r, pa, wa, q_in, n, d_shadow); \
        else hipLaunchKernelGGL((k_whitted_step<MODEV, LTV, SPHV>), dim3(grid_for(n)), dim3(kBlock), 0, stream, sc, r, pa, wa, q_in, n, d_shadow);   \
    } while (0)
#define GX_WH(LTV, SPHV) do { if (pl.wmode == WM_WHITTED) GX_WH2(WM_WHITTED, LTV, SPHV); else if (pl.wmode == WM_DIRECT_ONE) GX_WH2(WM_DIRECT_ONE, LTV, SPHV); else GX_WH2(WM_DIRECT_ALL, LTV, SPHV); } while (0)
        if (pl.area_only) { if (run.spheres) GX_WH(LT_AREA, true); else GX_WH(LT_AREA, false); }
        else { if (run.spheres) GX_WH(LT_ALL, true); else GX_WH(LT_ALL, false); }
#undef GX_WH
#undef GX_WH2
        ++run.launches;
        run.compact(COMPACT_FLAGS, q_in, n, st.pflags.p, 4, 3, &dctr->q_next, q_cur, st.queue_nee.p, st.queue_c0.p);
        if (run.timing) run.timer.end(stream);
        HIP_TRY(hipMemcpyAsync(run.s->h_counters, dctr, sizeof(Counters), hipMemcpyDeviceToHost, stream));
        HIP_TRY(hipStreamSynchronize(stream));
        if (int rc = compact_stalled(*run.s->h_counters)) return rc;
        n = (int)run.s->h_counters->q_next;
        n_shp = (int)run.s->h_counters->q_nee;
        n_cl = (int)run.s->h_counters->q_shadow;
        q_cl = st.queue_c0.p;
        q_in = q_cur;
        std::swap(q_cur, q_other);
        if (++guard > (1 << 20)) { set_error("path loop did not terminate"); return GNXR_ERR_INVALID; }
    }
    return GNXR_OK;
}

static int run_volpath_pass(RenderRun &run, long long u0, int kk) {
    gnxr_scene *s = run.s;
    RenderState &st = run.st;
// ... 53 lines not shown
            else { if (class_mask <= 1) GX_VS(LM_DIFFUSE, LT_ALL); else if (class_mask <= 3) GX_VS(LM_GLOSSY, LT_ALL); else GX_VS(LM_ALL, LT_ALL); }
#undef GX_VST
#undef GX_VS
#undef GX_VS_K
            run.launches += 2;
        }
        ++run.launches;
        run.compact(COMPACT_FLAGS, q_in, n, st.pflags.p, 4, 2, &dctr->q_next, q_cur, st.queue_nee.p, nullptr);
        if (run.timing) run.timer.end(stream);
        HIP_TRY(hipMemcpyAsync(s->h_counters, dctr, sizeof(Counters), hipMemcpyDeviceToHost, stream));
        HIP_TRY(hipStreamSynchronize(stream));
        if (int rc = compact_stalled(*s->h_counters)) return rc;
        n = (int)s->h_counters->q_next;
        n_media = (int)s->h_counters->q_nee;
        q_media = st.queue_nee.p;
        q_in = q_cur;
        std::swap(q_cur, q_other);
        if (Knobs::vol_pack() && n >= (1 << 16) && 2ll * n <= span) {
            const VolPackSet from = st.pack_set(in_alt), to = st.pack_set(!in_alt);
            hipLaunchKernelGGL(k_vol_pack, dim3(grid_for(n)), dim3(kBlock), 0, stream, q_in, n, from, to, st.vol_newslot.p);
            if (n_media > 0) hipLaunchKernelGGL(k_vol_remap, dim3(grid_for(n_media)), dim3(kBlock), 0, stream, st.queue_nee.p, n_media, (const int *)st.vol_newslot.p);
            run.launches += 2;
            in_alt = !in_alt;
            run.bind_set(to);
            q_in = nullptr;
            span = n;
        }
        if (++guard > (1 << 20)) { set_error("path loop did not terminate"); return GNXR_ERR_INVALID; }
    }
    if (in_alt) run.bind_set(st.pack_set(false));
    return GNXR_OK;
}

static int run_passes(RenderRun &run) {
    const RenderPlan &pl = run.pl;
    for (long long u0 = pl.unit_begin; u0 < pl.unit_end; u0 += pl.k) {
        const int kk = (int)std::min<long long>(pl.k, pl.unit_end - u0);
        run.raygen(run.pa, u0, kk, run.list_media ? run.st.pflags.p : nullptr);
        ++run.launches;
        if (int rc = pl.whitted ? run_whitted_pass(run, u0, kk) : run_volpath_pass(run, u0, kk)) return rc;
        PathArrays pr = run.pa;
        if (pl.volpath) pr.L = run.st.vol_Lout.p;
        run.resolve(pr, u0, kk);
        ++run.launches;
        ++run.passes;
        if (run.timing) { HIP_TRY(hipStreamSynchronize(run.stream)); run.timer.collect(); }
    }
    return GNXR_OK;
}

static void fill_stats(const RenderRun &run, double seconds_render, double seconds_total, gnxr_stats *stats) {
    const RenderPlan &pl = run.pl;
    const Counters &c = *run.s->h_counters;
    unsigned long long rays_closest = run.rays_closest, rays_any = run.rays_any, rays_mis = run.rays_mis, media_segments = run.media_segments;
    memset(stats, 0, sizeof(*stats));
    if (pl.path_int()) {
        rays_closest = run.new_paths + c.rays_continue + c.rays_mis;
        rays_any = c.rays_shadow;
        rays_mis = c.rays_mis;
    }
    if (pl.volpath) {
        rays_closest -= c.media_cont;
        media_segments -= c.media_cont;
    }
    stats->rays_closest = rays_closest + (pl.whitted ? c.whitted_mis : 0);
    stats->rays_any = pl.whitted ? c.whitted_shadow : rays_any;
    stats->camera_samples = run.src ? (uint64_t)run.src->n : (uint64_t)run.r.npix * pl.nsamples();
    stats->nodes_visited = c.nodes;
    stats->tris_tested = c.tris;
    stats->seconds_render = seconds_render;
    stats->seconds_total = seconds_total;
    stats->kernel_launches = run.launches;
    stats->passes = run.passes;
    stats->passes_in_flight = (uint32_t)pl.in_flight;
    stats->loop_iterations = run.loop_iterations;
    stats->state_bytes = RenderState::state_bytes(pl);
    stats->seconds_closest = run.timer.seconds[0]; stats->seconds_nee = run.timer.seconds[1]; stats->seconds_shade = run.timer.seconds[2];
    stats->seconds_trace = run.timer.seconds[0] + run.timer.seconds[1];
    stats->launches_closest = run.timer.launches[0]; stats->launches_nee = run.timer.launches[1];
    stats->rays_closest_nee = rays_mis;
    stats->media_segments = media_segments;
    stats->media_steps = c.media_steps;
    stats->leaf_retests = c.retests;
    stats->nodes_from_memory = c.nodes_global;
}

static int run_adaptive(RenderRun &run, RenderPlan &pl, PixelListSource &pix, void *d_rgba_out);
static void adaptive_stats(const PixelListSource &pix, gnxr_stats *stats);
static int render_one(gnxr_scene *s, const gnxr_render_params *pin, void *d_rgba_out, void *hip_stream, gnxr_stats *stats, bool reserve_only = false,
                      const RaySource *src = nullptr, const ViewSource *views = nullptr, PixelListSource *pix = nullptr, const FilmSource *film = nullptr) {
    if (!s || !pin || (!d_rgba_out && !src && !(film && film->accum))) { set_error("null argument"); return GNXR_ERR_INVALID; }
    RenderPlan pl;
    int rc = plan_render(s->cs, pin, src, views, pix, &pl);
    if (rc) return rc;
    const gnxr_render_params &p = pl.p;
    std::lock_guard<std::recursive_mutex> lock(s->render_mutex);
    if (int brc = s->bind()) return brc;
    auto t_start = std::chrono::steady_clock::now();
    hipStream_t stream = (hipStream_t)hip_stream;
    if ((rc = s->ensure_grid(p.light_strategy)) != GNXR_OK) return rc;
    DScene sc = s->device_scene(p.width, p.height);
    if ((rc = halton_index_bound(&sc.st.h, p.spp, pl.max_light_samples)) != GNXR_OK) return rc;
    if (pl.whitted) sc.materials = s->materials_single.p + 1;
    sc.escape_class = pl.escape_queue ? 3 : 0;
    DRender r;
    memset(&r, 0, sizeof(r));
    bool views_mixed_media = false;
    if (views) {
        s->h_view_cams.resize(std::max<size_t>(s->h_view_cams.size(), (size_t)views->n_views));
        make_view_cameras(views->cameras, views->media, views->n_views, p.width, p.height, s->h_view_cams.data());
        for (int v = 1; v < views->n_views; ++v) if (s->h_view_cams[v].medium != s->h_view_cams[0].medium) views_mixed_media = true;
        r.cam = s->h_view_cams[0];
    } else {
        r.cam = make_camera(s->cs.camera, p.width, p.height, s->cs.camera_medium);
    }
    r.W = p.width; r.H = p.height; r.spp = p.spp; r.max_depth = p.max_depth; r.rr_threshold = p.rr_threshold;
    r.shard_index = p.shard_index; r.shard_count = p.shard_count; r.shard_rows = p.shard_rows;
    r.npix = pl.npix;
    if (r.npix == 0) { if (stats) memset(stats, 0, sizeof(*stats)); return GNXR_OK; }
    {
        size_t free_b = 0, total_b = 0;
        const bool have_mem = hipMemGetInfo(&free_b, &total_b) == hipSuccess;
        if ((rc = pl.size_passes(s->st.L.n, have_mem, free_b)) != GNXR_OK) return rc;
    }
    if ((rc = s->st.reserve(pl)) != GNXR_OK) return rc;
    if (pix && (rc = s->st.reserve_adaptive(pl)) != GNXR_OK) return rc;
    if (pix && !s->h_ad_count && hipHostMalloc((void **)&s->h_ad_count, sizeof(unsigned int)) != hipSuccess) { s->h_ad_count = nullptr; set_error("hipHostMalloc failed"); return GNXR_ERR_OOM; }
    if (reserve_only) { if (stats) memset(stats, 0, sizeof(*stats)); return GNXR_OK; }

    RenderRun run(s, stream, pl, src, views, pix, sc, r);
    run.list_media = pl.volpath && (src || views_mixed_media);
    run.film = film;
    run.film_accum = film && film->accum ? film->accum : s->st.accum.p;
    if (views) HIP_TRY(hipMemcpyAsync(s->st.view_cams.p, s->h_view_cams.data(), (size_t)views->n_views * sizeof(DCamera), hipMemcpyHostToDevice, stream));
    if (!src) HIP_TRY(hipMemsetAsync(s->st.accum.p, 0, sizeof(float4) * r.npix, stream));
    if (film && film->accum && !film->keep) HIP_TRY(hipMemsetAsync(film->accum, 0, sizeof(float4) * r.npix, stream));
    HIP_TRY(hipMemsetAsync(run.dctr, 0, sizeof(Counters), stream));
    HIP_TRY(hipMemsetAsync(s->st.compact_ticket.p, 0, 2 * sizeof(unsigned int), stream));
    EventPair ev;
    HIP_TRY(hipEventCreate(&ev.a));
    HIP_TRY(hipEventCreate(&ev.b));
    HIP_TRY(hipEventRecord(ev.a, stream));
    if (pix) { if ((rc = run_adaptive(run, pl, *pix, d_rgba_out)) != GNXR_OK) return rc; }
    else if ((rc = pl.path_int() ? run_path_loop(run) : run_passes(run)) != GNXR_OK) return rc;
    if (film) {
        if (d_rgba_out) { hipLaunchKernelGGL(k_film_resolve, dim3(grid_for(r.npix)), dim3(kBlock), 0, stream, (const float4 *)run.film_accum, (long long)r.npix, (float4 *)d_rgba_out); ++run.launches; }
    } else if (!src && !pix) {
        hipLaunchKernelGGL(k_finish, dim3(grid_for(r.npix)), dim3(kBlock), 0, stream, r, (const float4 *)s->st.accum.p, (float4 *)d_rgba_out);
        ++run.launches;
    }
    HIP_TRY(hipEventRecord(ev.b, stream));
    HIP_TRY(hipMemcpyAsync(s->h_counters, run.dctr, sizeof(Counters), hipMemcpyDeviceToHost, stream));
    HIP_TRY(hipStreamSynchronize(stream));
    HIP_TRY(hipGetLastError());
    if (run.timing) run.timer.collect();
    if ((rc = compact_stalled(*s->h_counters)) != GNXR_OK) return rc;
    float ms = 0;
    HIP_TRY(hipEventElapsedTime(&ms, ev.a, ev.b));
    if (stats) fill_stats(run, ms * 1e-3, std::chrono::duration<double>(std::chrono::steady_clock::now() - t_start).count(), stats);
    if (stats && pix) adaptive_stats(*pix, stats);
    if (src && s->h_counters->li_bad) {
        set_error("gnxr_li_device: sample record %llu is out of range (px in [0, %d), py in [0, %d), s in [0, %d), medium in [-1, %d)); its L is (0, 0, 0, 0)",
                  ~s->h_counters->li_bad, p.width, p.height, p.spp, run.n_scene_media);
        return GNXR_ERR_INVALID;
    }
    return GNXR_OK;
}

// ... 84 lines not shown
```

### gnxraytracer_amd/csrc/kernels.hip.h

```cpp
#pragma once
#include "device_bsdf.h"
#include "device_lights.h"
#include "device_texture.h"

namespace gnxr {

constexpr int kBlock = 256;

constexpr int kRS = 2;
constexpr int kRSm = 2 * kRS;
constexpr int kRecGroups = 5;
struct PathArrays {
    float4 *ray_o;
    float4 *ray_d;
    float4 *beta;
    uint2 *meta;
    float4 *L;
    int *hit;
    unsigned char *pflags;
    unsigned char *pclass;
    float4 *sh_o;
    float4 *sh_d;
    float4 *sh_X;
    float4 *nbeta;
    float4 *mis_o;
    float4 *mis_d;
    float4 *mis_Y;
    unsigned int *nee_vis;
    __host__ __device__ void bind_records(float4 *const g[kRecGroups]) {
        ray_o = g[0]; ray_d = g[0] + 1; beta = g[1]; meta = reinterpret_cast<uint2 *>(g[1] + 1);
        sh_o = g[2]; sh_d = g[2] + 1; sh_X = g[3]; nbeta = g[3] + 1;
        mis_o = g[4]; mis_d = g[4] + 1;
    }
    __device__ void store_meta(size_t i, uint32_t x, uint32_t y) const { *reinterpret_cast<uint4 *>(&meta[i * kRSm]) = make_uint4(x, y, 0u, 0u); }
    __host__ __device__ PathArrays at(size_t base) const {
        PathArrays q = *this;
        q.ray_o += base * kRS; q.ray_d += base * kRS; q.beta += base * kRS; q.meta += base * kRSm;
        q.sh_o += base * kRS; q.sh_d += base * kRS; q.sh_X += base * kRS; q.nbeta += base * kRS;
        q.mis_o += base * kRS; q.mis_d += base * kRS;
        q.mis_Y += base; q.L += base; q.hit += base; q.pflags += base; q.pclass += base; q.nee_vis += base;
        return q;
    }
};

constexpr int kMaxRegions = 8;
struct Counters {
    unsigned long long nodes, tris;
    unsigned int q_next, q_nee, q_shadow, q_mis;
    unsigned int q_low;
    unsigned int q_class[4];
    unsigned int cursor;
    unsigned long long whitted_shadow;
    unsigned long long whitted_mis;
    unsigned long long media_steps;
    unsigned long long media_cont;
    unsigned long long retests;
    unsigned long long nodes_global;
    unsigned int n_queue;
    unsigned int iter;
    unsigned int region_lb[kMaxRegions + 1];
    unsigned int region_alive[kMaxRegions];
    unsigned long long rays_continue, rays_shadow, rays_mis;
    unsigned long long li_bad;
    unsigned int compact_stall;
    unsigned long long nee_applied_trace, nee_applied_sweep;
};

struct DScene {
    const float4 *nodes;
    const float4 *nodes4;
    int root4;
    const DTri *tris;
    const unsigned char *tri_class;
    const float4 *leaf_box;
    int leaf1_from_verts;
    const DSphere *spheres;
    int n_spheres;
    int escape_class;
    const DMaterial *materials;
    DLightTables lt;
    DSamplerTables st;
};

struct DRender {
    DCamera cam;
    int W, H, spp, max_depth;
    float rr_threshold;
    int shard_index, shard_count, shard_rows;
    int npix;
};

}
#include "compact_kernel.hip.h"
#include "trace_kernel.hip.h"
namespace gnxr {

GX_DEV void local_pixel(const DRender &r, int lp, int *x, int *y) {
    int row = lp / r.W;
    *x = lp - row * r.W;
    int blk = row / r.shard_rows;
    *y = (blk * r.shard_count + r.shard_index) * r.shard_rows + (row - blk * r.shard_rows);
}

GX_DEV void camera_ray(const DCamera &cam, const DSamplerTables &st, int px, int py, uint32_t index, V3 *o, V3 *d, float *tMax, int *dimOut) {
    SampleStream s(st, index, 0);
    float fx, fy, lx, ly;
    s.get2d(&fx, &fy);
    float pfx = (float)px + fx, pfy = (float)py + fy;
    s.dim += 1;
    if (cam.lens_radius > 0) s.get2d(&lx, &ly); else { s.dim += 2; lx = ly = 0.f; }
    V3 pCamera = xform_point(cam.r2c, V3(pfx, pfy, 0));
    V3 dir = normalize(V3(pCamera.x, pCamera.y, pCamera.z));
    V3 oc(0, 0, 0), dc = dir;
    if (cam.ortho) { oc = pCamera; dc = V3(0, 0, 1); }
    if (cam.lens_radius > 0) {
        float dx, dy;
        concentric_sample_disk(lx, ly, &dx, &dy);
        float plx = cam.lens_radius * dx, ply = cam.lens_radius * dy;
        float ft = cam.focal_distance / dc.z;
        V3 pFocus = oc + dc * ft;
        oc = V3(plx, ply, 0);
        dc = normalize(pFocus - oc);
    }
    const float *m = cam.c2w;
    float x = oc.x, y = oc.y, z = oc.z;
    float xp = (m[0] * x + m[1] * y) + (m[2] * z + m[3]);
    float yp = (m[4] * x + m[5] * y) + (m[6] * z + m[7]);
    float zp = (m[8] * x + m[9] * y) + (m[10] * z + m[11]);
    float wp = (m[12] * x + m[13] * y) + (m[14] * z + m[15]);
    float xAbs = (fabsf(m[0] * x) + fabsf(m[1] * y) + fabsf(m[2] * z) + fabsf(m[3]));
    float yAbs = (fabsf(m[4] * x) + fabsf(m[5] * y) + fabsf(m[6] * z) + fabsf(m[7]));
    float zAbs = (fabsf(m[8] * x) + fabsf(m[9] * y) + fabsf(m[10] * z) + fabsf(m[11]));
    V3 oError = GX_GAMMA(3) * V3(xAbs, yAbs, zAbs);
    V3 ow = (wp == 1) ? V3(xp, yp, zp) : V3((1.f / wp) * xp, (1.f / wp) * yp, (1.f / wp) * zp);
    V3 dw = xform_vector(m, dc);
    float lengthSquared = length_sq(dw);
    float tm = GX_INF;
    if (lengthSquared > 0) {
        float dt = dot(vabs(dw), oError) / lengthSquared;
        ow = ow + dw * dt;
        tm -= dt;
    }
    *o = ow; *d = dw; *tMax = tm; *dimOut = s.dim;
}

GX_DEV RayDiff camera_ray_diff(const DCamera &cam, const DSamplerTables &st, int px, int py, uint32_t index, int spp) {
    V3 o, d;
    float tMax;
    int dim;
    camera_ray(cam, st, px, py, index, &o, &d, &tMax, &dim);
    SampleStream s(st, index, 0);
    float fx, fy, lx, ly;
    s.get2d(&fx, &fy);
    s.dim += 1;
    if (cam.lens_radius > 0) s.get2d(&lx, &ly); else { s.dim += 2; lx = ly = 0.f; }
    V3 pCamera = xform_point(cam.r2c, V3((float)px + fx, (float)py + fy, 0));
    V3 dxCamera = xform_point(cam.r2c, V3(1, 0, 0)) - xform_point(cam.r2c, V3(0, 0, 0));
    V3 dyCamera = xform_point(cam.r2c, V3(0, 1, 0)) - xform_point(cam.r2c, V3(0, 0, 0));
    V3 rxO, ryO, rxD, ryD;
    if (cam.ortho) {
        V3 dxo = xform_vector(cam.r2c, V3(1, 0, 0)), dyo = xform_vector(cam.r2c, V3(0, 1, 0));
        if (cam.lens_radius > 0) {
            float ddx, ddy;
            concentric_sample_disk(lx, ly, &ddx, &ddy);
            float plx = cam.lens_radius * ddx, ply = cam.lens_radius * ddy;
            V3 pF0 = pCamera + V3(0, 0, 1) * (cam.focal_distance / 1.f);
            V3 dMain = normalize(pF0 - V3(plx, ply, 0));
            float ft = cam.focal_distance / dMain.z;
            V3 pFocus = pCamera + dxo + (ft * V3(0, 0, 1));
            rxO = V3(plx, ply, 0);
            rxD = normalize(pFocus - rxO);
            pFocus = pCamera + dyo + (ft * V3(0, 0, 1));
            ryO = V3(plx, ply, 0);
            ryD = normalize(pFocus - ryO);
        } else {
            rxO = pCamera + dxo;
            ryO = pCamera + dyo;
            rxD = ryD = V3(0, 0, 1);
        }
    } else if (cam.lens_radius > 0) {
        float ddx, ddy;
        concentric_sample_disk(lx, ly, &ddx, &ddy);
        float plx = cam.lens_radius * ddx, ply = cam.lens_radius * ddy;
        V3 dx = normalize(pCamera + dxCamera);
        float ft = cam.focal_distance / dx.z;
        V3 pFocus = V3(0, 0, 0) + (ft * dx);
        rxO = V3(plx, ply, 0);
        rxD = normalize(pFocus - rxO);
        V3 dy = normalize(pCamera + dyCamera);
        ft = cam.focal_distance / dy.z;
        pFocus = V3(0, 0, 0) + (ft * dy);
        ryO = V3(plx, ply, 0);
        ryD = normalize(pFocus - ryO);
    } else {
        rxO = ryO = V3(0, 0, 0);
        rxD = normalize(pCamera + dxCamera);
        ryD = normalize(pCamera + dyCamera);
    }
    RayDiff rdf;
    rdf.has = true;
    rdf.rxo = xform_point(cam.c2w, rxO);
    rdf.ryo = xform_point(cam.c2w, ryO);
    rdf.rxd = xform_vector(cam.c2w, rxD);
    rdf.ryd = xform_vector(cam.c2w, ryD);
    const float sc = 1 / gx_sqrt((float)(long long)spp);
    rdf.rxo = o + (rdf.rxo - o) * sc;
    rdf.ryo = o + (rdf.ryo - o) * sc;
    rdf.rxd = d + (rdf.rxd - d) * sc;
    rdf.ryd = d + (rdf.ryd - d) * sc;
    return rdf;
}

static __global__ void __launch_bounds__(kBlock) k_raygen(DScene sc, DRender r, PathArrays pa, int n_paths, int s0) {
    for (int slot = blockIdx.x * blockDim.x + threadIdx.x; slot < n_paths; slot += gridDim.x * blockDim.x) {
        int j = slot / r.npix;
        int lp = slot - j * r.npix;
        int px, py;
        local_pixel(r, lp, &px, &py);
        uint32_t index = halton_pixel_offset(sc.st.h, px, py) + (uint32_t)(s0 + j) * (uint32_t)sc.st.h.stride;
        V3 o, d;
        float tMax;
        int dim;
        camera_ray(r.cam, sc.st, px, py, index, &o, &d, &tMax, &dim);
        pa.ray_o[(size_t)slot * kRS] = make_float4(o.x, o.y, o.z, tMax);
        pa.ray_d[(size_t)slot * kRS] = make_float4(d.x, d.y, d.z, __int_as_float(r.cam.medium));
        pa.beta[(size_t)slot * kRS] = make_float4(1.f, 1.f, 1.f, 1.f);
        pa.L[slot] = make_float4(0.f, 0.f, 0.f, 0.f);
        pa.store_meta(slot, index, (uint32_t)dim);
    }
}

template <uint32_t LM, int LT>
GX_DEV int estimate_direct_record(const DScene &sc, const Bsdf<LM> &bsdf, const SurfacePoint &sp, V3 woN, int lightNum, float ul0, float ul1, float us0,
                                  float us1, const PathArrays &pa, size_t rec, float xw) {
    const int bsdfFlags = BSDF_ALL & ~BSDF_SPECULAR;
    int nflags = 0;
    V3 so, sd, mo, wi2;
    Spec X(0.f), Y(0.f);
    int expect = -1;
    LightSample ls = light_sample<LT>(sc.lt, lightNum, sp.p, ul0, ul1);
    float scatteringPdf = 0;
    if (ls.pdf > 0 && !ls.Li.is_black()) {
        Spec f = bsdf.f(woN, ls.wi, bsdfFlags) * absdot(ls.wi, sp.ns);
        scatteringPdf = bsdf.pdf(woN, ls.wi, bsdfFlags);
        if (!f.is_black()) {
            spawn_ray_to(sp.p, sp.pError, sp.n, ls.p1, ls.p1Error, ls.n1, &so, &sd);
            float weight = light_is_delta<LT>(sc.lt.lights[lightNum]) ? 1.f : power_heuristic(ls.pdf, scatteringPdf);
            X = f * ls.Li * weight / ls.pdf;
            nflags |= 1;
        }
    }
    if (!light_is_delta<LT>(sc.lt.lights[lightNum])) {
        int sampledType;
        Spec f = bsdf.sample_f(woN, &wi2, us0, us1, &scatteringPdf, bsdfFlags, &sampledType);
        f = f * absdot(wi2, sp.ns);
        bool sampledSpecular = (sampledType & BSDF_SPECULAR) != 0;
        if (!f.is_black() && scatteringPdf > 0) {
            float weight = 1;
            bool skip = false;
            if (!sampledSpecular) {
                float lightPdf = light_pdf<LT>(sc.lt, lightNum, sp.p, sp.pError, sp.n, wi2);
                if (lightPdf == 0) skip = true;
                else weight = power_heuristic(scatteringPdf, lightPdf);
            }
            if (!skip) {
                const DLight &lt = sc.lt.lights[lightNum];
                mo = offset_ray_origin(sp.p, sp.pError, sp.n, wi2);
                Spec Li2;
                if (LT == LT_AREA || lt.type == GNXR_LIGHT_AREA_TRI) {
                    V3 lp0(lt.p0[0], lt.p0[1], lt.p0[2]), lp1(lt.p1[0], lt.p1[1], lt.p1[2]), lp2(lt.p2[0], lt.p2[1], lt.p2[2]);
                    V3 ln = normalize(cross(lp0 - lp2, lp1 - lp2));
                    Li2 = area_L(lt, ln, -wi2);
                    expect = lt.tri_leaf;
                } else {
                    Li2 = light_Le<LT>(sc.lt, lightNum, mo, wi2);
                    expect = -1;
                }
                if (!Li2.is_black()) Y = f * Li2 * Spec(1.f) * weight / scatteringPdf;
                nflags |= 2;
            }
        }
    }
    if (nflags) {
        pa.sh_o[(size_t)rec * kRS] = make_float4(so.x, so.y, so.z, 1 - GX_SHADOW_EPS);
        pa.sh_d[(size_t)rec * kRS] = make_float4(sd.x, sd.y, sd.z, __int_as_float(nflags));
        pa.sh_X[(size_t)rec * kRS] = make_float4(X.r, X.g, X.b, xw);
        if (nflags & 2) {
            pa.mis_o[(size_t)rec * kRS] = make_float4(mo.x, mo.y, mo.z, __int_as_float(expect));
            pa.mis_d[(size_t)rec * kRS] = make_float4(wi2.x, wi2.y, wi2.z, 0.f);
            pa.mis_Y[rec] = make_float4(Y.r, Y.g, Y.b, 0.f);
        }
    }
    return nflags;
}
GX_DEV Spec nee_record_Ld(const PathArrays &pa, size_t rec, float *xw) {
    float4 sd4 = pa.sh_d[(size_t)rec * kRS], X4 = pa.sh_X[(size_t)rec * kRS];
    int flags = __float_as_int(sd4.w);
    Spec Ld(0.f);
    if ((flags & 1) && pa.sh_o[(size_t)rec * kRS].w == 1.f) Ld = Ld + Spec(X4.x, X4.y, X4.z);
    if (flags & 2) {
        float4 Y4 = pa.mis_Y[rec];
        Spec Y(Y4.x, Y4.y, Y4.z);
        if (pa.mis_o[(size_t)rec * kRS].w == 1.f && !Y.is_black()) Ld = Ld + Y;
    }
    *xw = X4.w;
    return Ld;
}

template <bool SPH, bool TEX, bool UV = false>
GX_DEV bool shade_hit_rebuild(const DScene &sc, const DMaterial *mats, int leaf, V3 ro, V3 rd, float tMax, V3 *p0, V3 *p1, V3 *p2, TriHit *h, int *triMat, int *triLight,
                              SurfacePoint *sp, V3 *sdpdu, V3 *sdpdv) {
    bool found = leaf != -1;
// ... 317 lines not shown
                                }
                            }
                            GX_STICK(7);
                            if (nflags || (MD == 2 && misSlot >= 0)) {
                                pa.sh_o[(size_t)path * kRS] = make_float4(so.x, so.y, so.z, 1 - GX_SHADOW_EPS);
                                pa.sh_d[(size_t)path * kRS] = make_float4(sd.x, sd.y, sd.z, __int_as_float(nflags));
                                pa.sh_X[(size_t)path * kRS] = make_float4(X.r, X.g, X.b, lightPdfSel);
                                if (nflags & 2) {
                                    pa.mis_o[(size_t)path * kRS] = make_float4(mo.x, mo.y, mo.z, __int_as_float(expect));
                                    pa.mis_d[(size_t)path * kRS] = make_float4(wi2.x, wi2.y, wi2.z, 0.f);
                                    pa.mis_Y[path] = make_float4(Y.r, Y.g, Y.b, 0.f);
                                }
                                pa.nbeta[(size_t)path * kRS] = make_float4(beta.r, beta.g, beta.b, 0.f);
                                const bool betaFinite = __builtin_isfinite(beta.r) && __builtin_isfinite(beta.g) && __builtin_isfinite(beta.b);
                                pa.nee_vis[path] = ((unsigned)nflags | (betaFinite ? 0u : 0x80u)) << 16;
                                wantNee = MD == 2 ? nflags != 0 : true;
                                if (MD == 2) misBits = (nflags & 1) | (betaFinite ? 2 : 0);
                                wantShadow = (nflags & 1) != 0;
                                wantMis = (nflags & 2) != 0;
                            }
                        }
                    }
                    GX_STICK(8);
                    V3 wo = -rd, wi;
                    float pdf, u0, u1;
                    int flags;
                    ss.get2d(&u0, &u1);
                    Spec f = bsdf.sample_f(wo, &wi, u0, u1, &pdf, BSDF_ALL, &flags);
                    if (!(f.is_black() || pdf == 0.f)) {
                        beta = beta * (f * absdot(wi, sp.ns) / pdf);
                        specularBounce = (flags & BSDF_SPECULAR) != 0;
                        if ((flags & BSDF_SPECULAR) && (flags & BSDF_TRANSMISSION)) {
                            float eta = mat->eta;
                            etaScale *= (dot(wo, sp.n) > 0) ? (eta * eta) : 1 / (eta * eta);
                        }
                        V3 o2 = offset_ray_origin(sp.p, sp.pError, sp.n, wi);
                        Spec rrBeta = beta * etaScale;
                        survive = true;
                        if (rrBeta.max_value() < r.rr_threshold && bounces > 3) {
                            float q = fmaxf(.05f, 1 - rrBeta.max_value());
                            if (ss.get1d() < q) survive = false;
                            else beta = beta / (1 - q);
                        }
                        if (survive) {
                            pa.ray_o[(size_t)path * kRS] = make_float4(o2.x, o2.y, o2.z, GX_INF);
                            pa.ray_d[(size_t)path * kRS] = make_float4(wi.x, wi.y, wi.z, d4.w);
                            pa.beta[(size_t)path * kRS] = make_float4(beta.r, beta.g, beta.b, etaScale);
                            pa.store_meta(path, index, (uint32_t)ss.dim | ((uint32_t)(bounces + 1) << 16) | (specularBounce ? 0x80000000u : 0u));
                        }
                    }
                }
            }
            GX_STICK(10);
        }
        pa.pflags[path] = (unsigned char)((survive ? 1 : 0) | (wantNee ? 2 : 0) | (wantShadow ? 4 : 0) | (wantMis ? 8 : 0));
        if (MD == 2 && misSlot >= 0) misList[26 * misCap + misSlot] = misBits | (survive ? 4 : 0);
        pathCur_ = pathNext_; leafCur_ = leafNext_; pathNext_ = pathNext2_;
    }
#ifdef GX_SHADE_STATS
    if ((threadIdx.x & 63) == 0) for (int k = 0; k < 16; ++k) if (sst_[k]) atomicAdd(&g_shade_stats[k], sst_[k]);
#endif
}

template <int LT>
__global__ void __launch_bounds__(kBlock) k_shade_escape(DScene sc, PathArrays pa, const int *__restrict__ queue, const unsigned int *n_dev) {
    const int n = (int)*n_dev;
    for (int i = blockIdx.x * blockDim.x + threadIdx.x; i < n; i += gridDim.x * blockDim.x) {
        const int path = queue[i];
        const uint2 m = pa.meta[(size_t)path * kRSm];
        const int bounces = (int)((m.y >> 16) & 0xffu);
        const bool specularBounce = (m.y >> 31) != 0;
        if (bounces == 0 || specularBounce) {
            const float4 o4 = pa.ray_o[(size_t)path * kRS], d4 = pa.ray_d[(size_t)path * kRS], b4 = pa.beta[(size_t)path * kRS], L4 = pa.L[path];
            const V3 ro(o4.x, o4.y, o4.z), rd(d4.x, d4.y, d4.z);
            const Spec beta(b4.x, b4.y, b4.z);
            Spec L(L4.x, L4.y, L4.z);
            for (int k = 0; k < sc.lt.n_infinite; ++k) L = L + beta * light_Le<LT>(sc.lt, sc.lt.infinite[k], ro, rd);
            pa.L[path] = make_float4(L.r, L.g, L.b, 0.f);
        }
        pa.pflags[path] = 0;
    }
}

static __global__ void __launch_bounds__(kBlock) k_queue_merge(const int *__restrict__ q_old, Counters *ctr, int first, int region, int base, int n_new, int *__restrict__ q_out) {
    const unsigned n_old = first ? 0u : ctr->q_next, split = first ? 0u : ctr->region_lb[region];
    const long long total = (long long)n_old + n_new;
    for (long long i = blockIdx.x * blockDim.x + threadIdx.x; i < total; i += (long long)gridDim.x * blockDim.x) {
        int v;
        if (i < split) v = q_old[i];
        else if (i < (long long)split + n_new) v = base + (int)(i - split);
        else v = q_old[i - n_new];
        q_out[i] = v;
    }
    if (blockIdx.x == 0 && threadIdx.x == 0) ctr->n_queue = (unsigned)total;
}

static __global__ void __launch_bounds__(64) k_loop_tail(const int *__restrict__ q_next, Counters *ctr, int n_regions, int region_size, unsigned iter) {
    __shared__ unsigned lb[kMaxRegions + 1];
    const unsigned n = ctr->q_next;
    const int r = threadIdx.x;
    if (r <= n_regions) {
        const long long key = (long long)r * region_size;
        unsigned lo = 0, hi = n;
        while (lo < hi) { const unsigned mid = (lo + hi) >> 1; if ((long long)q_next[mid] < key) lo = mid + 1; else hi = mid; }
        lb[r] = lo;
        ctr->region_lb[r] = lo;
    }
    __syncthreads();
    if (r < n_regions) ctr->region_alive[r] = lb[r + 1] - lb[r];
    if (r == 0) {
        ctr->rays_continue += n; ctr->rays_shadow += ctr->q_shadow; ctr->rays_mis += ctr->q_mis;
        ctr->n_queue = n;
        ctr->iter = iter;
    }
}

static __global__ void __launch_bounds__(kBlock) k_resolve(PathArrays pa, float4 *accum, int npix, int k) {
    for (int lp = blockIdx.x * blockDim.x + threadIdx.x; lp < npix; lp += gridDim.x * blockDim.x) {
        float4 a = accum[lp];
        for (int j = 0; j < k; ++j) {
            float4 l = pa.L[(size_t)j * npix + lp];
            a.x += l.x; a.y += l.y; a.z += l.z;
        }
        accum[lp] = a;
    }
}
static __global__ void __launch_bounds__(kBlock) k_finish(DRender r, const float4 *accum, float4 *out) {
    for (int lp = blockIdx.x * blockDim.x + threadIdx.x; lp < r.npix; lp += gridDim.x * blockDim.x) {
        int x, y;
        local_pixel(r, lp, &x, &y);
        float4 a = accum[lp];
        float spp = (float)(long long)r.spp;
        out[(size_t)y * r.W + x] = make_float4(a.x / spp, a.y / spp, a.z / spp, 1.f);
    }
}


GX_DEV gnxr_hit hit_record(const DScene &sc, V3 ro, V3 rd, int code, const TriHit &h) {
    gnxr_hit out;
    out.prim = -1; out.t = 0; out.b0 = out.b1 = out.b2 = 0; out.n[0] = out.n[1] = out.n[2] = 0;
    if (code < -1) {
        const int si = -2 - code;
        SurfacePoint sp = sphere_surface_point(sc.spheres[si], ro, rd, h.t, false);
        out.prim = sc.spheres[si].prim; out.t = h.t;
        out.n[0] = sp.n.x; out.n[1] = sp.n.y; out.n[2] = sp.n.z;
    }
    if (code >= 0) {
        const int leaf = code;
        V3 p0, p1, p2;
        load_tri(sc.tris, leaf, &p0, &p1, &p2);
        V3 nn = normalize(cross(p0 - p2, p1 - p2));
        const DTexTables &tt = tex_tables(sc.materials);
        if (tt.tri_n || tt.tri_s) {
            V3 dndu, dndv;
            SurfacePoint sp = surface_point_tables(tt, leaf, p0, p1, p2, h, false, &dndu, &dndv);
            if (sp.valid) nn = sp.n;
        }
        out.prim = sc.tris[leaf].prim; out.t = h.t; out.b0 = h.b0; out.b1 = h.b1; out.b2 = h.b2;
        out.n[0] = nn.x; out.n[1] = nn.y; out.n[2] = nn.z;
    }
    return out;
}
template <int STACK>
__global__ void __launch_bounds__(kBlock) k_trace_closest_api(DScene sc, const gnxr_ray *rays, long long n, gnxr_hit *hits) {
    __shared__ int stack[STACK * kBlock];
    TraceCounters tc = {0, 0};
    for (long long i = blockIdx.x * blockDim.x + threadIdx.x; i < n; i += (long long)gridDim.x * blockDim.x) {
        gnxr_ray r = rays[i];
        V3 ro(r.o[0], r.o[1], r.o[2]), rd(r.d[0], r.d[1], r.d[2]);
        TriHit h;
// ... 166 lines not shown
```

### gnxraytracer_amd/csrc/views_kernel.hip.h

```cpp
#pragma once
#include "kernels.hip.h"
#include "whitted_kernel.hip.h"

namespace gnxr {

GX_DEV void view_pixel(const DRender &r, int lp, int *view, int *px, int *py) {
    const int wh = r.W * r.H;
    const int v = lp / wh, p = lp - v * wh;
    const int y = p / r.W;
    *view = v; *px = p - y * r.W; *py = y;
}

static __global__ void __launch_bounds__(kBlock) k_raygen_views(DScene sc, DRender r, const DCamera *__restrict__ cams, PathArrays pa, int n_paths, int s0,
                                                                unsigned char *__restrict__ medium_keys) {
    for (int slot = blockIdx.x * blockDim.x + threadIdx.x; slot < n_paths; slot += gridDim.x * blockDim.x) {
        const int j = slot / r.npix;
        const int lp = slot - j * r.npix;
        int view, px, py;
        view_pixel(r, lp, &view, &px, &py);
        const DCamera cam = cams[view];
        uint32_t index = halton_pixel_offset(sc.st.h, px, py) + (uint32_t)(s0 + j) * (uint32_t)sc.st.h.stride;
        V3 o, d;
        float tMax;
        int dim;
        camera_ray(cam, sc.st, px, py, index, &o, &d, &tMax, &dim);
        pa.ray_o[(size_t)slot * kRS] = make_float4(o.x, o.y, o.z, tMax);
        pa.ray_d[(size_t)slot * kRS] = make_float4(d.x, d.y, d.z, __int_as_float(cam.medium));
        pa.beta[(size_t)slot * kRS] = make_float4(1.f, 1.f, 1.f, 1.f);
        pa.L[slot] = make_float4(0.f, 0.f, 0.f, 0.f);
        pa.store_meta(slot, index, (uint32_t)dim);
        if (medium_keys) medium_keys[slot] = cam.medium >= 0 ? 2 : 0;
    }
}

static __global__ void __launch_bounds__(kBlock) k_whitted_init_diff_views(DScene sc, DRender r, const DCamera *__restrict__ cams, PathArrays pa, WhittedArrays wa,
                                                                           int n_paths) {
    for (int slot = blockIdx.x * blockDim.x + threadIdx.x; slot < n_paths; slot += gridDim.x * blockDim.x) {
        int view, px, py;
        view_pixel(r, slot % r.npix, &view, &px, &py);
        const DCamera cam = cams[view];
        store_ray_diff(wa, (size_t)slot, camera_ray_diff(cam, sc.st, px, py, pa.meta[(size_t)slot * kRSm].x, r.spp));
    }
}

static __global__ void __launch_bounds__(kBlock) k_camera_rays(DSamplerTables st, DCamera cam, int W, int H, const int *__restrict__ px, const int *__restrict__ py,
                                                               const int *__restrict__ s, long long n, float4 *__restrict__ rays, int4 *__restrict__ samples,
                                                               unsigned long long *bad) {
    for (long long i = blockIdx.x * blockDim.x + threadIdx.x; i < n; i += (long long)gridDim.x * blockDim.x) {
        const int x = px[i], y = py[i], k = s[i];
        float4 ro = make_float4(0.f, 0.f, 0.f, 0.f), rd = ro;
        int4 rec = make_int4(0, 0, 0, 0);
        if (x >= 0 && x < W && y >= 0 && y < H && k >= 0) {
            uint32_t index = halton_pixel_offset(st.h, x, y) + (uint32_t)k * (uint32_t)st.h.stride;
            V3 o, d;
            float tMax;
            int dim;
            camera_ray(cam, st, x, y, index, &o, &d, &tMax, &dim);
            ro = make_float4(o.x, o.y, o.z, GX_INF);
            rd = make_float4(d.x, d.y, d.z, 0.f);
            rec = make_int4(x, y, k, cam.medium);
        } else {
            atomicMax(bad, ~(unsigned long long)i);
        }
        rays[2 * (size_t)i] = ro;
        rays[2 * (size_t)i + 1] = rd;
        samples[i] = rec;
    }
}

}
```

### include/gnxr.h

```cpp
#ifndef GNXR_H
#define GNXR_H

#include <stdint.h>

#ifdef __cplusplus
extern "C" {
#endif

#define GNXR_ABI_VERSION 5

typedef enum gnxr_status {
    GNXR_OK = 0,
    GNXR_ERR_INVALID = -1,
    GNXR_ERR_NO_DEVICE = -2,
    GNXR_ERR_OOM = -3,
    GNXR_ERR_UNSUPPORTED = -4,
    GNXR_ERR_IO = -5,
    GNXR_ERR_RUNTIME = -6
} gnxr_status;

typedef enum gnxr_material_type {
    GNXR_MAT_NONE = 0,
    GNXR_MAT_MATTE = 1,
    GNXR_MAT_MIRROR = 2,
// ... 204 lines not shown
    float t, b0, b1, b2;
    float n[3];
} gnxr_hit;
typedef struct gnxr_li_sample { int32_t px, py, s, medium; } gnxr_li_sample;
typedef struct gnxr_bsdf_result {
    float f[3];
    float pdf;
    float sample_f[3];
    float sample_pdf;
    float sample_wi[3];
    int32_t sampled_type;
    int32_t n_components;
    int32_t valid;
    float dudx, dvdy;
} gnxr_bsdf_result;
typedef struct gnxr_light_result {
    float Li[3];
    float pdf;
    float wi[3];
    float pdf_li;
    float pdf_select;
    float p_light[3];
} gnxr_light_result;

typedef struct gnxr_scene gnxr_scene;

int gnxr_abi_version(void);
int gnxr_abi_sizeof(int which);
int gnxr_init(int device_id);
int gnxr_init_devices(int32_t n_devices, const int32_t *device_ids);
void gnxr_shutdown(void);
const char *gnxr_last_error(void);
int gnxr_set_profiling(int flags);
int gnxr_probe_valu_peak(double *giga_wave_insts_per_s);
int gnxr_probe_gather_peak(double *giga_lane_loads_per_s);

int gnxr_scene_create(const gnxr_scene_desc *desc, gnxr_scene **out);
void gnxr_scene_destroy(gnxr_scene *scene);
int gnxr_scene_bvh(const gnxr_scene *scene, float *bounds6, int32_t *meta3, int32_t *ordered, int64_t node_capacity, int64_t *n_nodes);
int gnxr_scene_bvh4(const gnxr_scene *scene, void *nodes128, int64_t node_capacity, int64_t *n_nodes4, int32_t *root4, int32_t *stack_need);
int gnxr_scene_info(const gnxr_scene *scene, int32_t *n_bvh_nodes, int32_t *bvh_max_depth,
                    int32_t *n_light_voxels);
int gnxr_scene_update_vertices(gnxr_scene *scene, int32_t first_vertex, int32_t n_vertices, const float *xyz, void *hip_stream);
#define GNXR_UPDATE_MOVE_LIGHTS 1u
int gnxr_scene_update_vertices_ex(gnxr_scene *scene, int32_t first_vertex, int32_t n_vertices, const float *xyz, uint32_t flags, void *hip_stream);
int gnxr_scene_update_lights(gnxr_scene *scene, int32_t first_light, int32_t n_lights, const gnxr_light *lights);
int gnxr_scene_set_lights(gnxr_scene *scene, const gnxr_light *lights, int32_t n_lights, void *hip_stream);
int gnxr_scene_light_tables(gnxr_scene *scene, int32_t which, void *out, int64_t capacity_bytes, int64_t *n_bytes);
int gnxr_scene_update_environment(gnxr_scene *scene, const gnxr_light *light, const float *rgb, int32_t width, int32_t height, void *hip_stream);
int gnxr_scene_rebuild_bvh(gnxr_scene *scene, void *hip_stream);
typedef struct gnxr_geometry {
    int32_t struct_size;
    int32_t n_vertices, n_triangles;
    int32_t _pad;
    const float   *vertices;
    const int32_t *indices;
    const int32_t *tri_material;
    const int32_t *tri_light;
    const int32_t *tri_medium_inside;
    const int32_t *tri_medium_outside;
    const float   *tri_uv;
    const float   *tri_n;
    const float   *tri_s;
} gnxr_geometry;
int gnxr_scene_set_geometry(gnxr_scene *scene, const gnxr_geometry *g, void *hip_stream);
int gnxr_scene_update_materials(gnxr_scene *scene, int32_t first_material, int32_t n_materials, const gnxr_material *materials);
int gnxr_scene_set_triangle_materials(gnxr_scene *scene, int32_t first_triangle, int32_t n_triangles, const int32_t *material, void *hip_stream);
int gnxr_scene_triangle_materials(gnxr_scene *scene, int32_t *material_out, uint8_t *shade_class_out, int64_t capacity);
int gnxr_scene_env_tables(gnxr_scene *scene, int32_t which, void *out, int64_t capacity_bytes, int64_t *n_bytes);
int gnxr_scene_update_media(gnxr_scene *scene, int32_t first_medium, int32_t n_media, const gnxr_medium *media, const float *density, void *hip_stream);
int gnxr_scene_media_tables(gnxr_scene *scene, int32_t which, int32_t medium, void *out, int64_t capacity_bytes, int64_t *n_bytes);
int gnxr_scene_update_textures(gnxr_scene *scene, int32_t first_texture, int32_t n_textures, const gnxr_texture *textures, const float *texels, void *hip_stream);
int gnxr_scene_texture_tables(gnxr_scene *scene, int32_t which, int32_t texture, void *out, int64_t capacity_bytes, int64_t *n_bytes);
int gnxr_scene_set_camera(gnxr_scene *scene, const gnxr_camera *camera, int32_t camera_medium);

int gnxr_render(gnxr_scene *scene, const gnxr_render_params *params, float *rgba_out,
                gnxr_stats *stats);
int gnxr_render_device(gnxr_scene *scene, const gnxr_render_params *params, void *d_rgba_out,
                       void *hip_stream, gnxr_stats *stats);

int gnxr_render_reserve(gnxr_scene *scene, const gnxr_render_params *params);

int gnxr_scene_nee_apply_counts(gnxr_scene *scene, uint64_t *in_trace, uint64_t *by_sweep);

int gnxr_trace_closest(gnxr_scene *scene, const gnxr_ray *rays, int64_t n, gnxr_hit *hits);
int gnxr_trace_any(gnxr_scene *scene, const gnxr_ray *rays, int64_t n, uint8_t *occluded);
int gnxr_trace_closest_device(gnxr_scene *scene, const gnxr_ray *d_rays, int64_t n, gnxr_hit *d_hits, void *hip_stream);
int gnxr_trace_any_device(gnxr_scene *scene, const gnxr_ray *d_rays, int64_t n, uint8_t *d_occluded, void *hip_stream);

int gnxr_li_device(gnxr_scene *scene, const gnxr_render_params *params, const gnxr_ray *d_rays, const gnxr_li_sample *d_samples, int64_t n,
                   float *d_L, void *hip_stream, gnxr_stats *stats);

int gnxr_render_views_device(gnxr_scene *scene, const gnxr_render_params *params, const gnxr_camera *cameras, const int32_t *camera_media,
                             int32_t n_views, void *d_rgba_out, void *hip_stream, gnxr_stats *stats);
int gnxr_camera_rays_device(const gnxr_camera *camera, int32_t camera_medium, int32_t width, int32_t height, const int32_t *d_px,
                            const int32_t *d_py, const int32_t *d_s, int64_t n, gnxr_ray *d_rays, gnxr_li_sample *d_samples, void *hip_stream);

typedef struct gnxr_aov_buffers {
    float   *d_albedo;
    float   *d_normal;
    float   *d_shading_normal;
    float   *d_depth;
    int32_t *d_ids;
} gnxr_aov_buffers;
int gnxr_render_aov_device(gnxr_scene *scene, const gnxr_render_params *params, const gnxr_camera *cameras, const int32_t *camera_media,
                           int32_t n_views, const gnxr_aov_buffers *out, void *hip_stream, gnxr_stats *stats);
int gnxr_material_albedo(const gnxr_material *m, float rgb[3]);

typedef struct gnxr_adaptive_params { int32_t struct_size, min_spp, step_spp, guard; float threshold, floor; } gnxr_adaptive_params;
typedef struct gnxr_adaptive_info { int32_t struct_size, rounds; int64_t samples; int64_t pixels_at_budget; } gnxr_adaptive_info;
int gnxr_render_adaptive_device(gnxr_scene *scene, const gnxr_render_params *params, const gnxr_adaptive_params *adaptive, void *d_rgba_out,
                                int32_t *d_count_out, void *hip_stream, gnxr_stats *stats, gnxr_adaptive_info *info);

typedef struct gnxr_denoise_params { int32_t struct_size, width, height, n_views, iterations;
                                     float sigma_color, sigma_normal, sigma_depth; } gnxr_denoise_params;
typedef struct gnxr_denoise_buffers { int32_t struct_size, pad;
    const float *d_color;
    const float *d_color_b;
    const float *d_albedo;
    const float *d_normal;
    const float *d_depth;
} gnxr_denoise_buffers;
int gnxr_denoise_device(const gnxr_denoise_params *params, const gnxr_denoise_buffers *in, float *d_rgba_out, void *hip_stream);

enum { GNXR_FILTER_BOX = 0, GNXR_FILTER_TRIANGLE = 1, GNXR_FILTER_GAUSSIAN = 2, GNXR_FILTER_MITCHELL = 3, GNXR_FILTER_TABLE = 4 };
#define GNXR_FILM_CONTINUE 1u
typedef struct gnxr_film_filter { int32_t struct_size, kind; float radius_x, radius_y, a, b; const float *table; } gnxr_film_filter;
int gnxr_film_filter_table(const gnxr_film_filter *filter, float out[256]);
int gnxr_film_add_device(const gnxr_film_filter *filter, int32_t width, int32_t height, int32_t n_views, int32_t n_layers, const float *d_L,
                         const float *d_offsets, float *d_accum, void *hip_stream);
int gnxr_film_resolve_device(int32_t width, int32_t height, int32_t n_views, const float *d_accum, float *d_rgba_out, void *hip_stream);
int gnxr_render_filtered_device(gnxr_scene *scene, const gnxr_render_params *params, const gnxr_film_filter *filter, const gnxr_camera *cameras,
                                const int32_t *camera_media, int32_t n_views, void *d_rgba_out, float *d_accum, uint32_t flags, void *hip_stream,
                                gnxr_stats *stats);

#define GNXR_BAKE_FLIP_NORMALS 1u
typedef struct gnxr_bake_params { int32_t struct_size; uint32_t flags; int32_t dilate, medium; } gnxr_bake_params;
int gnxr_bake_texels_device(gnxr_scene *scene, const float *d_tri_lm_uv, int32_t width, int32_t height, int32_t *d_texel_tri, float *d_texel_bary,
                            void *hip_stream);
int gnxr_surface_rays_device(gnxr_scene *scene, int32_t width, int32_t height, const int32_t *d_tri, const float *d_bary, const int32_t *d_px,
                             const int32_t *d_py, const int32_t *d_s, int64_t n, uint32_t flags, int32_t medium, gnxr_ray *d_rays,
                             gnxr_li_sample *d_samples, float *d_pn, void *hip_stream);
int gnxr_bake_dilate_device(int32_t width, int32_t height, int32_t iterations, float *d_rgba, void *hip_stream);
int gnxr_bake_lightmap_device(gnxr_scene *scene, const gnxr_render_params *params, const gnxr_bake_params *bake, const float *d_tri_lm_uv,
                              void *d_rgba_out, void *hip_stream, gnxr_stats *stats);

#define GNXR_SH_CONTINUE 1u
typedef struct gnxr_lightprobe_params { int32_t struct_size; uint32_t flags; int32_t medium; } gnxr_lightprobe_params;
int gnxr_lightprobe_rays_device(gnxr_scene *scene, int32_t width, int32_t height, const float *d_pos, const int32_t *d_px, const int32_t *d_py,
                                const int32_t *d_s, int64_t n, int32_t medium, gnxr_ray *d_rays, gnxr_li_sample *d_samples, void *hip_stream);
int gnxr_sh_project_device(const gnxr_ray *d_rays, const float *d_L, int32_t n_probes, int64_t n_samples, float *d_sh_sum, uint32_t flags,
                           void *hip_stream);
int gnxr_bake_lightprobes_device(gnxr_scene *scene, const gnxr_render_params *params, const gnxr_lightprobe_params *probe_params,
                                 const float *d_positions, int32_t n_probes, void *d_sh_out, void *hip_stream, gnxr_stats *stats);
int gnxr_sh_irradiance_device(const float *d_sh, int32_t n_probes, const int32_t *d_probe, const float *d_normals, int64_t n, float *d_E,
                              void *hip_stream);

int gnxr_camera_matrices(const gnxr_camera *camera, int32_t width, int32_t height, float r2c[16], float c2w[16], float w2r[16]);
typedef struct gnxr_motion_params  { int32_t struct_size, width, height, n_views; } gnxr_motion_params;
typedef struct gnxr_motion_buffers { int32_t struct_size, pad;
    float   *d_motion;
    float   *d_guide;
    int32_t *d_prim;
} gnxr_motion_buffers;
int gnxr_motion_device(gnxr_scene *scene, const gnxr_motion_params *params, const gnxr_camera *cameras, const gnxr_camera *prev_cameras,
                       const float *d_prev_vertices, const gnxr_motion_buffers *out, void *hip_stream);
// ... 138 lines not shown
```

Before: 5413 Mrays/s.

## Cull camera rays missing the BVH root during raygen with adaptive fallback

Camera rays are tested against the root 4-wide BVH node in raygen, and rays that miss all root children are dropped before entering the path queue. Survivors are compacted per wave into a live list, which the queue-merge kernel prefix-sums and appends. A host-side check disables culling after the first batches if too few rays were culled to pay for the extra work. This adds a slab test, ballot compaction and a shared-memory prefix scan to raygen and merge.

```diff
diff --git a/gnxraytracer_amd/__init__.py b/gnxraytracer_amd/__init__.py
--- a/gnxraytracer_amd/__init__.py
+++ b/gnxraytracer_amd/__init__.py
@@ -318,6 +318,11 @@
         n, dmax, nv = C.c_int32(), C.c_int32(), C.c_int32()
         _check(lib().gnxr_scene_info(self._h, C.byref(n), C.byref(dmax), C.byref(nv)))
         return {"bvh_nodes": n.value, "bvh_max_depth": dmax.value, "light_voxels": nv.value}
+
+    def camera_rays_culled(self):
+        n = C.c_uint64()
+        _check(lib().gnxr_scene_camera_rays_culled(self._h, C.byref(n)))
+        return n.value
 
     def nee_apply_counts(self):
         t, w = C.c_uint64(), C.c_uint64()
@@ -1105,8 +1110,11 @@
     return r
 
 
-def stats_dict(s):
-    return {k: getattr(s, k) for k, _ in Stats._fields_}
+def stats_dict(s, scene=None):
+    d = {k: getattr(s, k) for k, _ in Stats._fields_}
+    if scene is not None:
+        d["camera_rays_culled"] = scene.camera_rays_culled()
+    return d
 
 
 class PathIntegrator:
@@ -1149,7 +1157,7 @@
         med = (C.c_int32 * max(V, 1))(*media) if media is not None else None
         st = Stats()
         _check(lib().gnxr_render_views_device(scene._h, C.byref(p), cams, med, V, _ptr(out), _addr(stream), C.byref(st)))
-        return out, stats_dict(st)
+        return out, stats_dict(st, scene)
 
     def RenderAdaptive(self, scene, width, height, spp, threshold, min_spp=16, step_spp=16, floor=0.01, guard=1, out=None, count_out=None, stream=None, **kw):
         import math
@@ -1297,7 +1305,7 @@
         img = np.zeros((height, width, 4), dtype=np.float32)
         st = Stats()
         _check(lib().gnxr_render(scene._h, C.byref(p), img.ctypes.data_as(C.POINTER(C.c_float)), C.byref(st)))
-        return img, stats_dict(st)
+        return img, stats_dict(st, scene)
 
     def Reserve(self, scene, width, height, spp, **kw):
         p = self.params(width, height, spp, **kw)
@@ -1308,7 +1316,7 @@
         st = Stats()
         _check(lib().gnxr_render_device(scene._h, C.byref(p), C.c_void_p(int(d_ptr)),
                                         C.c_void_p(int(stream) if stream else None), C.byref(st)))
-        return stats_dict(st)
+        return stats_dict(st, scene)
 
 
 class VolPathIntegrator(PathIntegrator):
diff --git a/gnxraytracer_amd/_abi.py b/gnxraytracer_amd/_abi.py
--- a/gnxraytracer_amd/_abi.py
+++ b/gnxraytracer_amd/_abi.py
@@ -259,6 +259,7 @@
     "gnxr_render_device": (C.c_int, [VP, P(RenderParams), VP, VP, P(Stats)]),
     "gnxr_render_reserve": (C.c_int, [VP, P(RenderParams)]),
     "gnxr_scene_nee_apply_counts": (C.c_int, [VP, P(u64), P(u64)]),
+    "gnxr_scene_camera_rays_culled": (C.c_int, [VP, P(u64)]),
     "gnxr_trace_closest": (C.c_int, [VP, P(Ray), i64, P(Hit)]),
     "gnxr_trace_any": (C.c_int, [VP, P(Ray), i64, P(u8)]),
     "gnxr_trace_closest_device": (C.c_int, [VP, VP, i64, VP, VP]),
diff --git a/gnxraytracer_amd/csrc/api.hip b/gnxraytracer_amd/csrc/api.hip
--- a/gnxraytracer_amd/csrc/api.hip
+++ b/gnxraytracer_amd/csrc/api.hip
@@ -207,6 +207,18 @@
     return GNXR_OK;
 }
 
+int gnxr_scene_camera_rays_culled(gnxr_scene *s, uint64_t *culled) {
+    if (!s) { set_error("null argument"); return GNXR_ERR_INVALID; }
+    std::lock_guard<std::recursive_mutex> lock(s->render_mutex);
+    uint64_t n = 0;
+    for (size_t i = 0; i <= s->replicas.size(); ++i) {
+        const Counters *c = s->copy(i)->h_counters;
+        if (c) n += c->camera_rays_culled;
+    }
+    if (culled) *culled = n;
+    return GNXR_OK;
+}
+
 int gnxr_render_device(gnxr_scene *s, const gnxr_render_params *pin, void *d_rgba_out, void *hip_stream, gnxr_stats *stats) {
     return render_sharded(s, pin, d_rgba_out, hip_stream, stats);
 }
diff --git a/gnxraytracer_amd/csrc/api_common.hip.h b/gnxraytracer_amd/csrc/api_common.hip.h
--- a/gnxraytracer_amd/csrc/api_common.hip.h
+++ b/gnxraytracer_amd/csrc/api_common.hip.h
@@ -74,6 +74,7 @@
     static int mis_defer_step() { const int v = env_int("GNXR_MIS_DEFER_STEP", 2); return v == 1 ? 1 : 2; }
     static int mis_defer_drain_at() { return std::max(1, std::min(64, env_int("GNXR_MIS_DEFER_DRAIN_AT", 64))); }
     static bool no_trace_nee_apply() { return env_set("GNXR_NO_TRACE_NEE_APPLY"); }
+    static bool no_raygen_cull() { return env_set("GNXR_NO_RAYGEN_CULL"); }
     static bool host_light_grid() { return env_set("GNXR_HOST_LIGHT_GRID"); }
     static bool binary_bvh() { return env_set("GNXR_BINARY_BVH"); }
     static long long closest_bin_min() { const char *e = getenv("GNXR_CLOSEST_BIN_MIN"); return e ? std::max(1ll, atoll(e)) : 65536ll; }
diff --git a/gnxraytracer_amd/csrc/api_render.hip.h b/gnxraytracer_amd/csrc/api_render.hip.h
--- a/gnxraytracer_amd/csrc/api_render.hip.h
+++ b/gnxraytracer_amd/csrc/api_render.hip.h
@@ -360,6 +360,8 @@
     const bool timing = (g_profiling & 1) != 0, count_wide = (g_profiling & 4) != 0, counting = (g_profiling & 2) != 0 && !count_wide;
     bool spheres;
     const int mis_mode = Knobs::no_mis_defer() ? 0 : Knobs::mis_defer_step(), mis_drain_at = Knobs::mis_defer_drain_at();
+    int raygen_mode = RAYGEN_PLAIN;
+    RaygenList raygen_list{nullptr, nullptr, 0, 0};
     bool list_media = false;
     int n_lights, n_scene_media;
     unsigned long long rays_closest = 0, rays_any = 0, rays_mis = 0, media_segments = 0;
@@ -377,6 +379,7 @@
                  const unsigned *n_dev = nullptr, unsigned kind_queue = 0x01010101u);
     int shade_stage(const int *q_in, int n, int *q_out, const unsigned *n_dev);
     void raygen(const PathArrays &at, long long u0, int kk, unsigned char *medium_keys);
+    int raygen_cull_mode() const;
     void resolve(const PathArrays &at, long long u0, int kk);
     void bind_set(const VolPackSet &ps);
 };
@@ -526,13 +529,34 @@
     return GNXR_OK;
 }
 
+int RenderRun::raygen_cull_mode() const {
+    const bool applies = pl.path_int() && !src && !pix && s->wide_ok && sc.root4 >= 0 && !counting && !spheres && sc.lt.n_infinite == 0;
+    return !applies ? RAYGEN_PLAIN : (Knobs::no_raygen_cull() ? RAYGEN_ALIVE : RAYGEN_CULL);
+}
 void RenderRun::raygen(const PathArrays &at, long long u0, int kk, unsigned char *medium_keys) {
     const int n_new = (int)(pl.unit * kk);
+    const int cn = count_wide ? 1 : 0;
+    int blocks = grid_for(n_new);
+    raygen_list = RaygenList{nullptr, nullptr, 0, 0};
+    if (raygen_mode != RAYGEN_PLAIN && !pix && (views || !src)) {
+        const int groups = (n_new + 63) / 64;
+        const int n_waves = std::min(std::min(groups, blocks * (kBlock / 64)), kMaxRaygenWaves);
+        raygen_list = RaygenList{st.queue_c0.p, reinterpret_cast<unsigned *>(st.queue_c1.p), n_waves, (groups + n_waves - 1) / n_waves * 64};
+        blocks = (n_waves + kBlock / 64 - 1) / (kBlock / 64);
+    }
+    const RaygenList ls = raygen_list;
+#define GX_RAYGEN(M) do { \
+        if (views) hipLaunchKernelGGL((k_raygen_views<M>), dim3(blocks), dim3(kBlock), 0, stream, sc, r, (const DCamera *)st.view_cams.p, at, n_new, (int)u0, medium_keys, ls, dctr, cn); \
+        else hipLaunchKernelGGL((k_raygen<M>), dim3(blocks), dim3(kBlock), 0, stream, sc, r, at, n_new, (int)u0, ls, dctr, cn); } while (0)
     if (pix) hipLaunchKernelGGL(k_raygen_pixels, dim3(grid_for(n_new)), dim3(kBlock), 0, stream, sc, r, at, pix->round, n_new, u0);
-    else if (views) hipLaunchKernelGGL(k_raygen_views, dim3(grid_for(n_new)), dim3(kBlock), 0, stream, sc, r, (const DCamera *)st.view_cams.p, at, n_new, (int)u0, medium_keys);
-    else if (!src) hipLaunchKernelGGL(k_raygen, dim3(grid_for(n_new)), dim3(kBlock), 0, stream, sc, r, at, n_new, (int)u0);
+    else if (views || !src) {
+        if (raygen_mode == RAYGEN_CULL) GX_RAYGEN(RAYGEN_CULL);
+        else if (raygen_mode == RAYGEN_ALIVE) GX_RAYGEN(RAYGEN_ALIVE);
+        else GX_RAYGEN(RAYGEN_PLAIN);
+    }
     else hipLaunchKernelGGL(k_raygen_rays, dim3(grid_for(n_new)), dim3(kBlock), 0, stream, sc, r, at, reinterpret_cast<const float4 *>(src->rays + u0),
                             reinterpret_cast<const int4 *>(src->samples + u0), n_new, n_scene_media, medium_keys, dctr, u0);
+#undef GX_RAYGEN
 }
 void RenderRun::resolve(const PathArrays &at, long long u0, int kk) {
     if (pix) hipLaunchKernelGGL(k_adaptive_accum, dim3(grid_for(pix->round.n_active)), dim3(kBlock), 0, stream, (const float4 *)at.L, pix->round, kk, u0, st.accum.p, st.ad_A.p);
@@ -573,6 +597,11 @@
     int *qbuf[2] = {st.queue_a.p, st.queue_b.p};
     int in_idx = 0;
     const int nee_in_trace = Knobs::no_trace_nee_apply() ? 0 : 1;
+    run.raygen_mode = run.raygen_cull_mode();
+    constexpr unsigned long long kCullPaysOneIn = 6;
+    struct Started { int iter; unsigned long long paths; };
+    std::vector<Started> started;
+    bool cull_decided = run.raygen_mode != RAYGEN_CULL;
     const unsigned *cnt_ptr = &dctr->n_queue;
     size_t next_sub = 0, done_subs = 0;
     int iter = 0, last_start = -(1 << 20), newest_seen = -1;
@@ -610,6 +639,12 @@
             }
         }
         if (done_subs == subs.size()) break;
+        if (!cull_decided && !started.empty() && newest_seen > started.front().iter) {
+            unsigned long long made = 0;
+            for (const Started &b : started) if (b.iter < newest_seen) made = b.paths;
+            if (kCullPaysOneIn * seen.camera_rays_culled < made) run.raygen_mode = RAYGEN_PLAIN;
+            cull_decided = true;
+        }
         bool any_active = false;
         long long n_upper = 0;
         for (int rg = 0; rg < R; ++rg) {
@@ -638,10 +673,12 @@
             const int n_new = (int)(pl.unit * nw.kk);
             const size_t base = (size_t)free_rg * half;
             run.raygen(run.pa.at(base), nw.u0, nw.kk, nullptr);
-            hipLaunchKernelGGL(k_queue_merge, dim3(grid_for(n_upper + n_new)), dim3(kBlock), 0, stream, (const int *)qbuf[out_idx], dctr, any_active ? 0 : 1, free_rg, (int)base, n_new, qbuf[in_idx]);
+            hipLaunchKernelGGL(k_queue_merge, dim3(grid_for(n_upper + n_new)), dim3(kBlock), 0, stream, (const int *)qbuf[out_idx], dctr, any_active ? 0 : 1, free_rg, (int)base, n_new, qbuf[in_idx],
+                               run.raygen_list);
             run.launches += 2;
             trace_idx = in_idx; n_trace_upper = n_upper + n_new;
             run.new_paths += (unsigned long long)n_new;
+            if (!cull_decided) started.push_back(Started{iter, run.new_paths});
             reg[free_rg].sub = (int)next_sub; reg[free_rg].started = iter; reg[free_rg].paths = n_new;
             last_start = iter;
             ++next_sub;
@@ -861,8 +898,7 @@
     stats->media_segments = media_segments;
     stats->media_steps = c.media_steps;
     stats->leaf_retests = c.retests;
-    stats->nodes_from_memory = c.nodes_global;
-}
+    stats->nodes_from_memory = c.nodes_global;}
 
 static int run_adaptive(RenderRun &run, RenderPlan &pl, PixelListSource &pix, void *d_rgba_out);
 static void adaptive_stats(const PixelListSource &pix, gnxr_stats *stats);
diff --git a/gnxraytracer_amd/csrc/kernels.hip.h b/gnxraytracer_amd/csrc/kernels.hip.h
--- a/gnxraytracer_amd/csrc/kernels.hip.h
+++ b/gnxraytracer_amd/csrc/kernels.hip.h
@@ -64,6 +64,7 @@
     unsigned long long li_bad;
     unsigned int compact_stall;
     unsigned long long nee_applied_trace, nee_applied_sweep;
+    unsigned long long camera_rays_culled;
 };
 
 struct DScene {
@@ -211,8 +212,98 @@
     return rdf;
 }
 
-static __global__ void __launch_bounds__(kBlock) k_raygen(DScene sc, DRender r, PathArrays pa, int n_paths, int s0) {
-    for (int slot = blockIdx.x * blockDim.x + threadIdx.x; slot < n_paths; slot += gridDim.x * blockDim.x) {
+GX_DEV bool ray_misses_root4(const DScene &sc, V3 o, V3 d, float tMax) {
+    const float4 *q = sc.nodes4 + 8 * (size_t)sc.root4;
+    const V3 inv(1.f / d.x, 1.f / d.y, 1.f / d.z);
+    const int neg0 = inv.x < 0, neg1 = inv.y < 0, neg2 = inv.z < 0;
+    const float4 nX = q[neg0 ? 3 : 0], fX = q[neg0 ? 0 : 3], nY = q[neg1 ? 4 : 1], fY = q[neg1 ? 1 : 4], nZ = q[neg2 ? 5 : 2], fZ = q[neg2 ? 2 : 5];
+    const float k = 1 + 2 * GX_GAMMA(3);
+    unsigned hitMask = 0;
+    if (!(__builtin_isinf(inv.x) || __builtin_isinf(inv.y) || __builtin_isinf(inv.z))) {
+#define GX_ROOT_SLAB3(C, BIT)                                                                                \
+    {                                                                                                        \
+        const float e = fmaxf(fmaxf((nX.C - o.x) * inv.x, (nY.C - o.y) * inv.y), (nZ.C - o.z) * inv.z);      \
+        const float x = fminf(fminf((fX.C - o.x) * inv.x, (fY.C - o.y) * inv.y), (fZ.C - o.z) * inv.z) * k;  \
+        hitMask |= (e <= x && e < tMax && x > 0.f) ? (BIT) : 0u;                                             \
+    }
+        GX_ROOT_SLAB3(x, 1u) GX_ROOT_SLAB3(y, 2u) GX_ROOT_SLAB3(z, 4u) GX_ROOT_SLAB3(w, 8u)
+#undef GX_ROOT_SLAB3
+    } else {
+#define GX_ROOT_SLAB(C, BIT)                                                              \
+    {                                                                                     \
+        float tMin = (nX.C - o.x) * inv.x, tMx = (fX.C - o.x) * inv.x;                    \
+        float tyMin = (nY.C - o.y) * inv.y, tyMax = (fY.C - o.y) * inv.y;                 \
+        tMx *= k; tyMax *= k;                                                             \
+        bool ok = !(tMin > tyMax || tyMin > tMx);                                         \
+        if (tyMin > tMin) tMin = tyMin;                                                   \
+        if (tyMax < tMx) tMx = tyMax;                                                     \
+        float tzMin = (nZ.C - o.z) * inv.z, tzMax = (fZ.C - o.z) * inv.z;                 \
+        tzMax *= k;                                                                       \
+        ok = ok && !(tMin > tzMax || tzMin > tMx);                                        \
+        if (tzMin > tMin) tMin = tzMin;                                                   \
+        if (tzMax < tMx) tMx = tzMax;                                                     \
+        ok = ok && (tMin < tMax) && (tMx > 0);                                            \
+        hitMask |= ok ? (BIT) : 0u;                                                       \
+    }
+        GX_ROOT_SLAB(x, 1u) GX_ROOT_SLAB(y, 2u) GX_ROOT_SLAB(z, 4u) GX_ROOT_SLAB(w, 8u)
+#undef GX_ROOT_SLAB
+    }
+    return hitMask == 0;
+}
+
+enum RaygenMode { RAYGEN_PLAIN = 0, RAYGEN_ALIVE = 1, RAYGEN_CULL = 2 };
+
+constexpr int kMaxRaygenWaves = 8192;
+struct RaygenList {
+    int *live;
+    unsigned *counts;
+    int n_waves, chunk;
+};
+
+template <int MODE>
+GX_DEV bool raygen_store(const DScene &sc, const PathArrays &pa, int slot, V3 o, V3 d, float tMax, int medium, uint32_t index, int dim) {
+    const bool culled = MODE == RAYGEN_CULL && ray_misses_root4(sc, o, d, tMax);
+    pa.L[slot] = make_float4(0.f, 0.f, 0.f, 0.f);
+    if (!culled) {
+        pa.ray_o[(size_t)slot * kRS] = make_float4(o.x, o.y, o.z, tMax);
+        pa.ray_d[(size_t)slot * kRS] = make_float4(d.x, d.y, d.z, __int_as_float(medium));
+        pa.beta[(size_t)slot * kRS] = make_float4(1.f, 1.f, 1.f, 1.f);
+        pa.store_meta(slot, index, (uint32_t)dim);
+    }
+    return culled;
+}
+
+template <int MODE, typename F>
+GX_DEV void raygen_slots(int n_paths, const RaygenList &ls, Counters *ctr, int count_nodes, F ray) {
+    if (MODE == RAYGEN_PLAIN) {
+        for (int slot = blockIdx.x * blockDim.x + threadIdx.x; slot < n_paths; slot += gridDim.x * blockDim.x) ray(slot);
+        return;
+    }
+    const int wave = blockIdx.x * (kBlock / 64) + (threadIdx.x >> 6), lane = __lane_id();
+    if (wave >= ls.n_waves) return;
+    const long long first = (long long)wave * ls.chunk;
+    unsigned run = 0, n_culled = 0;
+    for (int t = 0; t < ls.chunk && first + t < n_paths; t += 64) {
+        const long long slot = first + t + lane;
+        bool alive = false;
+        if (slot < n_paths) alive = !ray((int)slot);
+        const unsigned long long m = __ballot(alive), v = __ballot(slot < n_paths);
+        if (alive) ls.live[first + run + (unsigned)__popcll(m & ((1ull << lane) - 1ull))] = (int)slot;
+        run += (unsigned)__popcll(m);
+        n_culled += (unsigned)__popcll(v & ~m);
+    }
+    if (lane == 0) {
+        ls.counts[wave] = run;
+        if (MODE == RAYGEN_CULL && n_culled != 0) {
+            atomicAdd(&ctr->camera_rays_culled, (unsigned long long)n_culled);
+            if (count_nodes) atomicAdd(&ctr->nodes, (unsigned long long)n_culled);
+        }
+    }
+}
+
+template <int MODE>
+__global__ void __launch_bounds__(kBlock) k_raygen(DScene sc, DRender r, PathArrays pa, int n_paths, int s0, RaygenList ls, Counters *ctr, int count_nodes) {
+    raygen_slots<MODE>(n_paths, ls, ctr, count_nodes, [&](int slot) -> bool {
         int j = slot / r.npix;
         int lp = slot - j * r.npix;
         int px, py;
@@ -222,12 +313,8 @@
         float tMax;
         int dim;
         camera_ray(r.cam, sc.st, px, py, index, &o, &d, &tMax, &dim);
-        pa.ray_o[(size_t)slot * kRS] = make_float4(o.x, o.y, o.z, tMax);
-        pa.ray_d[(size_t)slot * kRS] = make_float4(d.x, d.y, d.z, __int_as_float(r.cam.medium));
-        pa.beta[(size_t)slot * kRS] = make_float4(1.f, 1.f, 1.f, 1.f);
-        pa.L[slot] = make_float4(0.f, 0.f, 0.f, 0.f);
-        pa.store_meta(slot, index, (uint32_t)dim);
-    }
+        return raygen_store<MODE>(sc, pa, slot, o, d, tMax, r.cam.medium, index, dim);
+    });
 }
 
 template <uint32_t LM, int LT>
@@ -711,10 +798,39 @@
     }
 }
 
-static __global__ void __launch_bounds__(kBlock) k_queue_merge(const int *__restrict__ q_old, Counters *ctr, int first, int region, int base, int n_new, int *__restrict__ q_out) {
+static __global__ void __launch_bounds__(kBlock) k_queue_merge(const int *__restrict__ q_old, Counters *ctr, int first, int region, int base, int n_new, int *__restrict__ q_out,
+                                                               RaygenList ls) {
+    __shared__ unsigned pre[kMaxRaygenWaves + 1];
+    __shared__ unsigned part[kBlock];
     const unsigned n_old = first ? 0u : ctr->q_next, split = first ? 0u : ctr->region_lb[region];
+    const long long stride = (long long)gridDim.x * blockDim.x, t0 = blockIdx.x * blockDim.x + threadIdx.x;
+    if (ls.live) {
+        const int per = (ls.n_waves + kBlock - 1) / kBlock, w0 = threadIdx.x * per;
+        unsigned sum = 0;
+        for (int w = w0; w < w0 + per && w < ls.n_waves; ++w) sum += ls.counts[w];
+        part[threadIdx.x] = sum;
+        __syncthreads();
+        if (threadIdx.x == 0) {
+            unsigned run = 0;
+            for (int k = 0; k < kBlock; ++k) { const unsigned v = part[k]; part[k] = run; run += v; }
+            pre[ls.n_waves] = run;
+        }
+        __syncthreads();
+        unsigned run = part[threadIdx.x];
+        for (int w = w0; w < w0 + per && w < ls.n_waves; ++w) { pre[w] = run; run += ls.counts[w]; }
+        __syncthreads();
+        const unsigned n_live = pre[ls.n_waves];
+        for (long long i = t0; i < n_old; i += stride) q_out[i < split ? i : i + n_live] = q_old[i];
+        const unsigned n_slots = (unsigned)ls.n_waves * (unsigned)ls.chunk;
+        for (unsigned t = (unsigned)t0; t < n_slots; t += (unsigned)stride) {
+            const unsigned w = t / (unsigned)ls.chunk, j = t - w * (unsigned)ls.chunk;
+            if (j < pre[w + 1] - pre[w]) q_out[(size_t)split + pre[w] + j] = base + ls.live[t];
+        }
+        if (t0 == 0) ctr->n_queue = n_old + n_live;
+        return;
+    }
     const long long total = (long long)n_old + n_new;
-    for (long long i = blockIdx.x * blockDim.x + threadIdx.x; i < total; i += (long long)gridDim.x * blockDim.x) {
+    for (long long i = t0; i < total; i += stride) {
         int v;
         if (i < split) v = q_old[i];
         else if (i < (long long)split + n_new) v = base + (int)(i - split);
diff --git a/gnxraytracer_amd/csrc/views_kernel.hip.h b/gnxraytracer_amd/csrc/views_kernel.hip.h
--- a/gnxraytracer_amd/csrc/views_kernel.hip.h
+++ b/gnxraytracer_amd/csrc/views_kernel.hip.h
@@ -11,9 +11,10 @@
     *view = v; *px = p - y * r.W; *py = y;
 }
 
-static __global__ void __launch_bounds__(kBlock) k_raygen_views(DScene sc, DRender r, const DCamera *__restrict__ cams, PathArrays pa, int n_paths, int s0,
-                                                                unsigned char *__restrict__ medium_keys) {
-    for (int slot = blockIdx.x * blockDim.x + threadIdx.x; slot < n_paths; slot += gridDim.x * blockDim.x) {
+template <int MODE>
+__global__ void __launch_bounds__(kBlock) k_raygen_views(DScene sc, DRender r, const DCamera *__restrict__ cams, PathArrays pa, int n_paths, int s0,
+                                                         unsigned char *__restrict__ medium_keys, RaygenList ls, Counters *ctr, int count_nodes) {
+    raygen_slots<MODE>(n_paths, ls, ctr, count_nodes, [&](int slot) -> bool {
         const int j = slot / r.npix;
         const int lp = slot - j * r.npix;
         int view, px, py;
@@ -24,13 +25,9 @@
         float tMax;
         int dim;
         camera_ray(cam, sc.st, px, py, index, &o, &d, &tMax, &dim);
-        pa.ray_o[(size_t)slot * kRS] = make_float4(o.x, o.y, o.z, tMax);
-        pa.ray_d[(size_t)slot * kRS] = make_float4(d.x, d.y, d.z, __int_as_float(cam.medium));
-        pa.beta[(size_t)slot * kRS] = make_float4(1.f, 1.f, 1.f, 1.f);
-        pa.L[slot] = make_float4(0.f, 0.f, 0.f, 0.f);
-        pa.store_meta(slot, index, (uint32_t)dim);
         if (medium_keys) medium_keys[slot] = cam.medium >= 0 ? 2 : 0;
-    }
+        return raygen_store<MODE>(sc, pa, slot, o, d, tMax, cam.medium, index, dim);
+    });
 }
 
 static __global__ void __launch_bounds__(kBlock) k_whitted_init_diff_views(DScene sc, DRender r, const DCamera *__restrict__ cams, PathArrays pa, WhittedArrays wa,
diff --git a/include/gnxr.h b/include/gnxr.h
--- a/include/gnxr.h
+++ b/include/gnxr.h
@@ -310,6 +310,8 @@
 int gnxr_render_reserve(gnxr_scene *scene, const gnxr_render_params *params);
 
 int gnxr_scene_nee_apply_counts(gnxr_scene *scene, uint64_t *in_trace, uint64_t *by_sweep);
+
+int gnxr_scene_camera_rays_culled(gnxr_scene *scene, uint64_t *culled);
 
 int gnxr_trace_closest(gnxr_scene *scene, const gnxr_ray *rays, int64_t n, gnxr_hit *hits);
 int gnxr_trace_any(gnxr_scene *scene, const gnxr_ray *rays, int64_t n, uint8_t *occluded);
```

Result: no change. 5449 Mrays/s, median of 6 (+0.7%).
